# CodyRichter/MLMicroserviceTemplate

Hardware: AMD Instinct MI355X
Metric: requests/sec (whole node) + p50 latency, ResNet-50 bs=32 (higher is better)
Workload: dtype bf16; 1 GPU; model=resnet50-v1.5, global_batch=32, per_gpu_batch=32, image_size=224, parallelism=dp1, backend=fused, concurrent_slots=True, cu_partitions=2, hipgraph=True, inflight=4, numa_bound=True, partition_mode=intra, prestage=False, ranks_consistent=True, dist_backend=none, dist_world=1

## Files before the change

### mlmicroservicetemplate_amd/models/resnet.py

```python
from __future__ import annotations

import math
import os
from dataclasses import dataclass
from typing import Dict, List, Optional, Tuple

import torch
import torch.nn.functional as F

STAGES: Tuple[Tuple[int, int, int, int], ...] = (
    (3, 64, 256, 1),
    (4, 128, 512, 2),
    (6, 256, 1024, 2),
    (3, 512, 2048, 2),
)
IMAGENET_MEAN = (0.485 * 255, 0.456 * 255, 0.406 * 255)
IMAGENET_STD = (0.229 * 255, 0.224 * 255, 0.225 * 255)
NUM_CLASSES = 1000
CHAIN_CONV2_DEFAULT = ((64, 256, 64), (0, 256, 64))


@dataclass
class ConvSpec:
    name: str
    cin: int
    cout: int
    k: int
    stride: int
    pad: int


def conv_specs() -> List[ConvSpec]:
    specs = [ConvSpec("stem", 3, 64, 7, 2, 3)]
    cin = 64
    for si, (nblocks, mid, cout, stride) in enumerate(STAGES):
        for bi in range(nblocks):
            s = stride if bi == 0 else 1
            p = f"layer{si + 1}.{bi}"
            specs.append(ConvSpec(p + ".conv1", cin, mid, 1, 1, 0))
            specs.append(ConvSpec(p + ".conv2", mid, mid, 3, s, 1))
            specs.append(ConvSpec(p + ".conv3", mid, cout, 1, 1, 0))
            if bi == 0:
                specs.append(ConvSpec(p + ".down", cin, cout, 1, s, 0))
            cin = cout
    return specs


def init_resnet50(seed: int = 0, num_classes: int = NUM_CLASSES) -> Dict[str, torch.Tensor]:
    g = torch.Generator().manual_seed(seed)
    params: Dict[str, torch.Tensor] = {}
    for spec in conv_specs():
        fan_in = spec.cin * spec.k * spec.k
        w = torch.randn(spec.cout, spec.cin, spec.k, spec.k, generator=g) * math.sqrt(2.0 / fan_in)
        params[spec.name + ".w"] = w
        c = spec.cout
        params[spec.name + ".bn.gamma"] = 0.5 + 0.5 * torch.rand(c, generator=g)
        params[spec.name + ".bn.beta"] = 0.1 * torch.randn(c, generator=g)
        params[spec.name + ".bn.mean"] = 0.1 * torch.randn(c, generator=g)
        params[spec.name + ".bn.var"] = 0.5 + torch.rand(c, generator=g)
    params["fc.w"] = torch.randn(num_classes, 2048, generator=g) * math.sqrt(1.0 / 2048)
    params["fc.b"] = 0.01 * torch.randn(num_classes, generator=g)
    return params


_BN = {"weight": "gamma", "bias": "beta", "running_mean": "mean", "running_var": "var"}


def torchvision_name(k: str) -> Optional[str]:
    if k.endswith("num_batches_tracked"):
        return None
    p = k.split(".")
    if p[0] == "conv1":
        return "stem.w"
    if p[0] == "bn1":
        return f"stem.bn.{_BN[p[1]]}"
    if p[0] == "fc":
        return {"weight": "fc.w", "bias": "fc.b"}[p[1]]
    if p[0].startswith("layer") and len(p) >= 4:
        blk = f"{p[0]}.{p[1]}"
        if p[2].startswith("conv"):
            return f"{blk}.{p[2]}.w"
        if p[2].startswith("bn"):
            return f"{blk}.conv{p[2][2:]}.bn.{_BN[p[3]]}"
        if p[2] == "downsample":
            return f"{blk}.down.w" if p[3] == "0" else f"{blk}.down.bn.{_BN[p[4]]}"
    return k


def load_resnet50(path: str, num_classes: int = NUM_CLASSES) -> Dict[str, torch.Tensor]:
    from ..utils.checkpoint import load_validated

    spec = {k: (tuple(v.shape), torch.float32) for k, v in init_resnet50_spec(num_classes).items()}
    return load_validated(path, spec, rename=lambda k: k if k in spec else torchvision_name(k))


def init_resnet50_spec(num_classes: int = NUM_CLASSES) -> Dict[str, torch.Tensor]:
    out: Dict[str, torch.Tensor] = {}
    for spec in conv_specs():
        out[spec.name + ".w"] = torch.empty(spec.cout, spec.cin, spec.k, spec.k, device="meta")
        for n in ("gamma", "beta", "mean", "var"):
            out[f"{spec.name}.bn.{n}"] = torch.empty(spec.cout, device="meta")
    out["fc.w"] = torch.empty(num_classes, 2048, device="meta")
    out["fc.b"] = torch.empty(num_classes, device="meta")
    return out


BN_EPS = 1e-5


def fold_bn(params: Dict[str, torch.Tensor], name: str) -> Tuple[torch.Tensor, torch.Tensor]:
    gamma = params[name + ".bn.gamma"]
    beta = params[name + ".bn.beta"]
    mean = params[name + ".bn.mean"]
    var = params[name + ".bn.var"]
    scale = gamma / torch.sqrt(var + BN_EPS)
    bias = beta - mean * scale
    return scale, bias


def normalize_reference(images_u8_nhwc: torch.Tensor) -> torch.Tensor:
    x = images_u8_nhwc.float()
    mean = torch.tensor(IMAGENET_MEAN, device=x.device)
    std = torch.tensor(IMAGENET_STD, device=x.device)
    x = (x - mean) / std
    return x.permute(0, 3, 1, 2).contiguous()


def _ref_conv_bn(params, x, spec: ConvSpec, relu: bool, residual=None):
    y = F.conv2d(x, params[spec.name + ".w"], stride=spec.stride, padding=spec.pad)
    y = F.batch_norm(
        y,
        params[spec.name + ".bn.mean"],
        params[spec.name + ".bn.var"],
        params[spec.name + ".bn.gamma"],
        params[spec.name + ".bn.beta"],
        training=False,
        eps=BN_EPS,
    )
    if residual is not None:
        y = y + residual
    return F.relu(y) if relu else y


def resnet50_reference(params: Dict[str, torch.Tensor], images_u8_nhwc: torch.Tensor) -> torch.Tensor:
    specs = {s.name: s for s in conv_specs()}
    x = normalize_reference(images_u8_nhwc)
    x = _ref_conv_bn(params, x, specs["stem"], relu=True)
    x = F.max_pool2d(x, kernel_size=3, stride=2, padding=1)
    for si, (nblocks, _mid, _cout, _stride) in enumerate(STAGES):
        for bi in range(nblocks):
            p = f"layer{si + 1}.{bi}"
            identity = x
            if bi == 0:
                identity = _ref_conv_bn(params, x, specs[p + ".down"], relu=False)
            y = _ref_conv_bn(params, x, specs[p + ".conv1"], relu=True)
            y = _ref_conv_bn(params, y, specs[p + ".conv2"], relu=True)
            x = _ref_conv_bn(params, y, specs[p + ".conv3"], relu=True, residual=identity)
    x = x.mean(dim=(2, 3))
    return F.linear(x, params["fc.w"], params["fc.b"])


class ResNet50Eager(torch.nn.Module):

    def __init__(self, params: Dict[str, torch.Tensor], device, dtype=torch.bfloat16, fold: bool = True):
        super().__init__()
        self.specs = {s.name: s for s in conv_specs()}
        self.fold = fold
        self.dtype = dtype
        self.w: Dict[str, torch.Tensor] = {}
        self.sb: Dict[str, Tuple[torch.Tensor, torch.Tensor]] = {}
        for s in conv_specs():
            w = params[s.name + ".w"]
            scale, bias = fold_bn(params, s.name)
            if fold:
                w = w * scale.view(-1, 1, 1, 1)
            self.w[s.name] = w.to(device=device, dtype=dtype).contiguous(memory_format=torch.channels_last)
            self.sb[s.name] = (scale.to(device=device, dtype=dtype), bias.to(device=device, dtype=dtype))
        self.fc_w = params["fc.w"].to(device=device, dtype=dtype)
        self.fc_b = params["fc.b"].to(device=device, dtype=dtype)
        self.mean = torch.tensor(IMAGENET_MEAN, device=device, dtype=torch.float32)
        self.inv_std = 1.0 / torch.tensor(IMAGENET_STD, device=device, dtype=torch.float32)

    @torch.no_grad()
    def update_params(self, params: Dict[str, torch.Tensor]) -> None:
        for s in conv_specs():
            w = params[s.name + ".w"]
            scale, bias = fold_bn(params, s.name)
            if self.fold:
                w = w * scale.view(-1, 1, 1, 1)
            self.w[s.name].copy_(w)
            self.sb[s.name][0].copy_(scale)
            self.sb[s.name][1].copy_(bias)
        self.fc_w.copy_(params["fc.w"])
        self.fc_b.copy_(params["fc.b"])

    def _cbr(self, x, name, relu=True, residual=None):
        s = self.specs[name]
        y = F.conv2d(x, self.w[name], stride=s.stride, padding=s.pad)
        scale, bias = self.sb[name]
        if self.fold:
            y = y + bias.view(1, -1, 1, 1)
        else:
            y = y * scale.view(1, -1, 1, 1) + bias.view(1, -1, 1, 1)
        if residual is not None:
            y = y + residual
        return F.relu(y) if relu else y

    @torch.no_grad()
    def forward(self, images_u8_nhwc: torch.Tensor) -> torch.Tensor:
        x = ((images_u8_nhwc.float() - self.mean) * self.inv_std).to(self.dtype)
        x = x.permute(0, 3, 1, 2)
        x = self._cbr(x, "stem")
        x = F.max_pool2d(x, 3, 2, 1)
        for si, (nblocks, _m, _c, _s) in enumerate(STAGES):
            for bi in range(nblocks):
                p = f"layer{si + 1}.{bi}"
                identity = self._cbr(x, p + ".down", relu=False) if bi == 0 else x
                y = self._cbr(x, p + ".conv1")
                y = self._cbr(y, p + ".conv2")
                x = self._cbr(y, p + ".conv3", residual=identity)
        x = x.mean(dim=(2, 3))
        return F.linear(x, self.fc_w, self.fc_b)


def conv_shapes(image_size: int = 224) -> List[Tuple[ConvSpec, int, int]]:
    out: List[Tuple[ConvSpec, int, int]] = []
    block_in = cur = image_size
    for s in conv_specs():
        if s.name.endswith(".conv1"):
            block_in = cur
        hin = block_in if s.name.endswith(".down") else cur
        ho = (hin + 2 * s.pad - s.k) // s.stride + 1
        out.append((s, hin, ho))
        if s.name == "stem":
            cur = (ho + 2 - 3) // 2 + 1
        elif not s.name.endswith(".down"):
            cur = ho
    return out


def resnet50_flops_per_image(image_size: int = 224) -> float:
    total = 0.0
    for s, _hin, ho in conv_shapes(image_size):
        total += 2.0 * ho * ho * s.cout * s.cin * s.k * s.k
    return total + 2.0 * 2048 * NUM_CLASSES


class ResNet50Fused:

    def __init__(self, params: Dict[str, torch.Tensor], device, max_batch: int = 256,
                 tuning: Optional[Dict[str, Tuple[int, int]]] = None, image_size: int = 224):
        from .. import ops

        self.ops = ops
        self.device = torch.device(device)
        self.image_size = image_size
        self.tuning = dict(tuning or {})
        self.specs = {s.name: s for s in conv_specs()}
        self.w: Dict[str, torch.Tensor] = {}
        self.b: Dict[str, torch.Tensor] = {}
        for s in conv_specs():
            scale, bias = fold_bn(params, s.name)
            w = params[s.name + ".w"] * scale.view(-1, 1, 1, 1)
            self.w[s.name] = ops.pack_conv_weight(w).to(self.device)
            self.b[s.name] = bias.to(device=self.device, dtype=torch.float32).contiguous()
        self.dual_w: Dict[str, torch.Tensor] = {}
        self.dual_b: Dict[str, torch.Tensor] = {}
        for si, (_nb, _m, _c, _s) in enumerate(STAGES):
            p0 = f"layer{si + 1}.0"
            w3, wd = self.w[p0 + ".conv3"], self.w[p0 + ".down"]
            self.dual_w[p0] = torch.cat([w3.reshape(w3.shape[0], -1), wd.reshape(wd.shape[0], -1)], 1).contiguous()
            self.dual_b[p0] = (self.b[p0 + ".conv3"] + self.b[p0 + ".down"]).contiguous()
        self.fuse_down = True
        self.chain = os.environ.get("MLS_CHAIN", "1") != "0"
        self.chain_skip: set = {b for b in os.environ.get("MLS_CHAIN_SKIP", "").split(",") if b}
        mode = os.environ.get("MLS_CHAIN_CONV2", "1")
        self.chain_conv2 = mode != "0"
        self.chain_conv2_shapes = ops.CHAIN_CONV2_SHAPES if mode == "2" else CHAIN_CONV2_DEFAULT
        self.chain_conv2_skip: set = {b for b in os.environ.get("MLS_CHAIN_CONV2_SKIP", "").split(",") if b}
        self.chain_l3 = os.environ.get("MLS_CHAIN_L3", "0") == "1"
        if os.environ.get("MLS_CHAIN_L2_CW"):
            ops.set_chain_l2_cw(int(os.environ["MLS_CHAIN_L2_CW"]))
        if os.environ.get("MLS_CHAIN_L2_BM"):
            ops.lib().mls_chain_set_l2_bm(int(os.environ["MLS_CHAIN_L2_BM"]))
        if os.environ.get("MLS_CHAIN_VARIANT"):
            ops.lib().mls_chain_set_variant(int(os.environ["MLS_CHAIN_VARIANT"]))
        self.fuse_stem = image_size == 224 and os.environ.get("MLS_FUSED_STEM", "1") != "0"
        self.fuse_stem_conv1 = os.environ.get("MLS_STEM_CONV1", "0") == "1"
        self.fc_w = params["fc.w"].to(device=self.device, dtype=torch.bfloat16).contiguous()
        self.fc_b = params["fc.b"].to(device=self.device, dtype=torch.float32).contiguous()
        self.num_classes = self.fc_w.shape[0]
        self.mean = IMAGENET_MEAN
        self.std = IMAGENET_STD
        self.max_batch = max_batch
        self._ws = ops.StreamWorkspace(self._workspace_bytes(max_batch) // 4 + 1, self.device)
        self.fuse_head = os.environ.get("MLS_FUSED_HEAD", "1") != "0"
        self._pool = ops.StreamWorkspace(max_batch * self.fc_w.shape[1], self.device, zero=True)

    @property
    def workspace(self) -> torch.Tensor:
        return self._ws.get()

    @torch.no_grad()
    def update_params(self, params: Dict[str, torch.Tensor]) -> None:
        from .. import ops

        for s in conv_specs():
            scale, bias = fold_bn(params, s.name)
            w = ops.pack_conv_weight(params[s.name + ".w"] * scale.view(-1, 1, 1, 1))
            self.w[s.name].copy_(w)
            self.b[s.name].copy_(bias)
        for si in range(len(STAGES)):
            p0 = f"layer{si + 1}.0"
            w3, wd = self.w[p0 + ".conv3"], self.w[p0 + ".down"]
            self.dual_w[p0].copy_(torch.cat([w3.reshape(w3.shape[0], -1), wd.reshape(wd.shape[0], -1)], 1))
            self.dual_b[p0].copy_(self.b[p0 + ".conv3"] + self.b[p0 + ".down"])
        self.fc_w.copy_(params["fc.w"])
        self.fc_b.copy_(params["fc.b"])

    def layer_gemm_shapes(self, batch: int) -> List[Tuple[str, int, int, int]]:
        out = []
        for s, _hin, ho in conv_shapes(self.image_size):
            k = s.k * 32 if s.name == "stem" else s.k * s.k * s.cin
            out.append((s.name, batch * ho * ho, s.cout, k))
            if s.name.endswith(".0.down"):
                c3 = self.specs[s.name[: -len("down")] + "conv3"]
                out.append((s.name[: -len("down")] + "dual", batch * ho * ho, s.cout, c3.cin + s.cin))
        out.append(("fc", batch, self.num_classes, 2048))
        return out

    def _plan(self, name: str, M: int, N: int, K: int) -> Tuple[int, int]:
        if name in self.tuning:
            return self.tuning[name]
        return self.ops.gemm_heuristic(M, N, K)

    def _workspace_bytes(self, batch: int) -> int:
        need = 0
        for b in sorted({1, 2, 4, 8, 16, 32, 64, 128, 256, batch}):
            if b > batch:
                continue
            for name, M, N, K in self.layer_gemm_shapes(b):
                cfg, sk = self._plan(name, M, N, K)
                if cfg in self.ops.PIPE_CFGS:
                    sk = sk % 16 or 1
                if sk > 1:
                    need = max(need, sk * M * N * 4)
        return max(need, batch * NUM_CLASSES * 4, 1 << 20)

    def _conv(self, x, name, act, residual=None, pad=None):
        s = self.specs[name]
        cfg, sk = self.tuning.get(name, (0, 0))
        return self.ops.conv2d_nhwc(x, self.w[name], self.b[name], kernel=s.k, stride=s.stride,
                                    pad=s.pad if pad is None else pad,
                                    residual=residual, act=act, workspace=self.workspace, cfg=cfg, splitk=sk)


    def _chained(self, p: str, nxt: str, dual: bool) -> bool:
        if not self.chain or p in self.chain_skip:
            return False
        c3 = self.specs[p + ".conv3"]
        k = c3.cin + (self.specs[p + ".down"].cin if dual else 0)
        c1 = self.specs[nxt + ".conv1"]
        shape = (k, c3.cout, c1.cout)
        if shape == (256, 1024, 256) and not self.chain_l3:
            return False
        return c1.k == 1 and c1.stride == 1 and shape in self.ops.CHAIN_SHAPES

    def _conv2_fused(self, p: str, nxt: str, dual: bool, t1: torch.Tensor) -> bool:
        if not self.chain_conv2 or p in self.chain_conv2_skip:
            return False
        c2, c3 = self.specs[p + ".conv2"], self.specs[p + ".conv3"]
        kb = self.specs[p + ".down"].cin if dual else 0
        shape = (kb, c3.cout, self.specs[nxt + ".conv1"].cout)
        return (c2.k == 3 and c2.stride == 1 and c2.pad == 1 and c2.cin == 64 and c2.cout == 64
                and shape in self.chain_conv2_shapes and t1.shape[2] <= self.ops.CHAIN_CONV2_MAX_W)

    def forward(self, images_u8_nhwc: torch.Tensor) -> torch.Tensor:
        ops = self.ops
        B = images_u8_nhwc.shape[0]
        if self.fuse_head:
            pooled = self._trunk(images_u8_nhwc, pool=True)
            _v, _i, logits = ops.fc_head(pooled, self.fc_w, self.fc_b, 0, logits=self._logits_buf(B))
            return logits.to(torch.bfloat16)
        x = self._trunk(images_u8_nhwc, pool=False)
        pooled = ops.avgpool_global_nhwc(x)
        cfg, sk = self.tuning.get("fc", (0, 0))
        return ops.gemm(pooled, self.fc_w, self.fc_b, workspace=self.workspace, cfg=cfg, splitk=sk)

    __call__ = forward

    def _logits_buf(self, B: int) -> torch.Tensor:
        return self.workspace[: B * self.num_classes].view(B, self.num_classes)

    def classify(self, images_u8_nhwc: torch.Tensor, k: int = 5, err: Optional[torch.Tensor] = None):
        if self.fuse_head:
            pooled = self._trunk(images_u8_nhwc, pool=True)
            B = images_u8_nhwc.shape[0]
            vals, idx, _ = self.ops.fc_head(pooled, self.fc_w, self.fc_b, k, logits=self._logits_buf(B), err=err)
            return vals, idx
        vals, idx = self.ops.softmax_topk(self.forward(images_u8_nhwc), k)
        if err is not None:
            bad = (err[: idx.shape[0]] != 0).view(-1, 1)
            idx = torch.where(bad, torch.full_like(idx, -1), idx)
            vals = torch.where(bad, torch.full_like(vals, float("nan")), vals)
        return vals, idx

    def _trunk(self, images_u8_nhwc: torch.Tensor, pool: bool) -> torch.Tensor:
        ops = self.ops
        B = images_u8_nhwc.shape[0]
        if B > self.max_batch:
            raise ValueError(f"batch {B} > max_batch {self.max_batch}")
        if self.fuse_stem and self.fuse_stem_conv1:
            x, t1 = ops.stem_pool_u8(images_u8_nhwc, self.w["stem"], self.b["stem"], self.mean, self.std,
                                     conv1_w=self.w["layer1.0.conv1"], conv1_b=self.b["layer1.0.conv1"])
        else:
            if self.fuse_stem:
                x = ops.stem_pool_u8(images_u8_nhwc, self.w["stem"], self.b["stem"], self.mean, self.std)
            else:
                x = ops.normalize_u8(images_u8_nhwc, self.mean, self.std, pad=3)
                x = self._conv(x, "stem", ops.ACT_RELU, pad=0)
                x = ops.maxpool2d_nhwc(x, 3, 2, 1)
            t1 = self._conv(x, "layer1.0.conv1", ops.ACT_RELU)
        blocks = [(si, bi) for si, (nblocks, _m, _c, _s) in enumerate(STAGES) for bi in range(nblocks)]
        for idx, (si, bi) in enumerate(blocks):
            p = f"layer{si + 1}.{bi}"
            nxt = f"layer{blocks[idx + 1][0] + 1}.{blocks[idx + 1][1]}" if idx + 1 < len(blocks) else None
            dual = bi == 0 and self.fuse_down
            chained = nxt is not None and self._chained(p, nxt, dual)
            if chained and self._conv2_fused(p, nxt, dual, t1):
                w1n, b1n = self.w[nxt + ".conv1"], self.b[nxt + ".conv1"]
                w1n = w1n.reshape(w1n.shape[0], -1)
                w2, b2 = self.w[p + ".conv2"], self.b[p + ".conv2"]
                if dual:
                    x, t1 = ops.conv3x3_chain(t1, w2, b2, self.dual_w[p], self.dual_b[p], w1n, b1n, a2=x,
                                              stride2=self.specs[p + ".down"].stride)
                else:
                    w3 = self.w[p + ".conv3"]
                    x, t1 = ops.conv3x3_chain(t1, w2, b2, w3.reshape(w3.shape[0], -1), self.b[p + ".conv3"], w1n,
                                              b1n, residual=x)
                continue
            t2 = self._conv(t1, p + ".conv2", ops.ACT_RELU)
            if chained:
                w1n, b1n = self.w[nxt + ".conv1"], self.b[nxt + ".conv1"]
                w1n = w1n.reshape(w1n.shape[0], -1)
                if dual:
                    x, t1 = ops.conv1x1_chain(t2, self.dual_w[p], self.dual_b[p], w1n, b1n, a2=x,
                                              stride2=self.specs[p + ".down"].stride)
                else:
                    w3 = self.w[p + ".conv3"]
                    x, t1 = ops.conv1x1_chain(t2, w3.reshape(w3.shape[0], -1), self.b[p + ".conv3"], w1n, b1n,
                                              residual=x)
                continue
            if dual:
                cfg, sk = self.tuning.get(p + ".dual", (0, 0))
                x = ops.conv1x1_dual(t2, x, self.dual_w[p], self.dual_b[p], stride2=self.specs[p + ".down"].stride,
                                     act=ops.ACT_RELU, workspace=self.workspace, cfg=cfg, splitk=sk)
            else:
                identity = self._conv(x, p + ".down", ops.ACT_NONE) if bi == 0 else x
                if nxt is None and pool:
                    pooled = self._pool.get()[: B * self.fc_w.shape[1]].view(B, -1)
                    cfg, _sk = self.tuning.get(p + ".conv3", (0, 0))
                    s3 = self.specs[p + ".conv3"]
                    ops.conv2d_pool(t2, self.w[p + ".conv3"], self.b[p + ".conv3"], pooled, kernel=s3.k,
                                    stride=s3.stride, pad=s3.pad, residual=identity, act=ops.ACT_RELU, cfg=cfg)
                    return pooled
                x = self._conv(t2, p + ".conv3", ops.ACT_RELU, residual=identity)
            if nxt is not None:
                t1 = self._conv(x, nxt + ".conv1", ops.ACT_RELU)
        if pool:
            pooled = self._pool.get()[: B * self.fc_w.shape[1]].view(B, -1)
            pooled.copy_(ops.avgpool_global_nhwc(x).float())
            return pooled
        return x
```

### mlmicroservicetemplate_amd/ops/__init__.py

```python
from __future__ import annotations

from . import _lib
from ._lib import NativeError, available, check, lib, stream_ptr
from ._core import (
    ACT_GELU,
    ACT_NONE,
    ACT_RELU,
    ACT_SILU,
    ACT_SILU_MUL,
    ACT_TANH,
    StreamWorkspace,
    conv_out_hw,
)
from .tables import (
    gemm_plan,
    gemm_tile_plan,
    load_blas_tuning,
    small_m_plan_for,
    tile_cfg_for,
    tile_route_for,
)
from .gemm_ops import (
    FP8_MAX,
    GEMM_TILE_CFGS,
    SPLIT_COUNTER_ELEMS,
    fold_layernorm,
    fold_norm,
    fp8_reference,
    gemm,
    gemm_heuristic,
    gemm_rmsnorm,
    gemm_tile,
    gemm_tile_ln,
    layernorm_from_partials,
    ln_partials,
    interleave_gate_up,
    pack_skinny,
    pack_skinny_fp8,
    pack_skinny_reference,
    silu_mul_interleaved,
    skinny_fp8,
    mgemm,
    skinny_packed,
    skinny_packed_ar,
    split_counters,
)
from .dispatch import (
    BLAS_MIN_M,
    TILE_MIN_M,
    mgemm_route,
    linear_add_rmsnorm,
    linear,
    linear_ln,
    ln_foldable,
)
from .softmax import (
    softmax_rows,
    softmax_topk,
    topk_large,
)
from .vision import (
    CFG_HALO,
    CFG_HALO_N32,
    CFG_HALO_XL,
    CFG_PIPE,
    CHAIN_CONV2_MAX_W,
    CHAIN_CONV2_SHAPES,
    CHAIN_SHAPES,
    HALO_CFGS,
    PIPE_CFGS,
    PIPE_VARIANTS,
    avgpool_global_nhwc,
    bn_act,
    conv1x1_chain,
    conv1x1_dual,
    conv2d_nhwc,
    conv2d_pool,
    conv3x3_halo,
    conv3x3_halo_geometry,
    conv3x3_chain,
    conv3x3_pipe,
    conv3x3_pipe_geometry,
    fc_head,
    maxpool2d_nhwc,
    normalize_u8,
    pack_conv_weight,
    set_chain_l2_cw,
    stem_pool_u8,
)
from .transformer import (
    DecodePartials,
    decode_attention,
    decode_attention_fp8,
    decode_pick,
    embed_layernorm,
    embed_layernorm_packed,
    embedding,
    flash_attention,
    flash_attention_ctx,
    flash_attention_rows,
    kv_append,
    last_rows,
    layernorm,
    prefill_slots,
    rmsnorm,
    rope_,
    rope_kv_,
    rope_kv_fp8_,
    skinny_packed_combine,
    skinny_packed_combine_ar,
)
from .image import (
    IMAGE_CONTAINER_BYTES,
    IMAGE_SCRATCH_PER_IMAGE,
    d2h_push,
    gpu_sleep,
    h2d_pull,
    h2d_pull_cell,
    image_decode,
)
from .partition import (
    MASK_WORDS,
    census_cus,
    cu_census,
    cu_masked_stream,
    intra_partition_words,
    partition_masks,
    xcd_cu_masks,
)

__all__ = [
    "NativeError",
    "available",
    "lib",
    "conv2d_nhwc",
    "gemm",
    "normalize_u8",
    "maxpool2d_nhwc",
    "avgpool_global_nhwc",
    "bn_act",
    "softmax_topk",
    "softmax_rows",
    "pack_conv_weight",
    "conv_out_hw",
    "gemm_heuristic",
]
```

### mlmicroservicetemplate_amd/ops/_lib.py

```python
from __future__ import annotations

import ctypes
import os
import threading
from typing import Optional

import torch

from . import build as _build

_c = ctypes
_LOCK = threading.Lock()
_LIB: Optional[ctypes.CDLL] = None

P = _c.c_void_p
I = _c.c_int
L = _c.c_long
F = _c.c_float
SZ = _c.c_size_t
FP = _c.POINTER(_c.c_float)

_SIGS = {
    "mls_conv2d": [P, P, P, P, P, P, P, SZ, I, I, I, I, I, I, I, I, I, I, I, I, P],
    "mls_conv2d_dual": [P, P, P, P, P, P, SZ, I, I, I, I, I, I, I, I, I, I, I, I, P],
    "mls_conv_chain": [P, P, P, P, P, P, P, P, P, I, I, I, I, I, I, I, I, I, I, P],
    "mls_conv_chain_conv2": [P, P, P, P, P, P, P, P, P, P, P, I, I, I, I, I, I, I, I, I, I, P],
    "mls_gemm": [P, P, P, P, P, P, P, SZ, I, I, I, I, I, I, P],
    "mls_gemm_heuristic": [I, I, I, _c.POINTER(I), _c.POINTER(I)],
    "mls_gemm_tile": [P, P, P, P, P, I, I, I, I, I, I, I, I, I, P, _c.c_longlong, P, I, P],
    "mls_gemm_tile_pick": [I, I],
    "mls_gemm_tile_ln": [P, P, P, P, P, I, I, I, I, I, P, P, P, P, _c.c_longlong, F, P],
    "mls_gemm_num_cfgs": [],
    "mls_normalize_u8": [P, P, I, I, I, I, FP, FP, P],
    "mls_maxpool2d": [P, P, I, I, I, I, I, I, I, P],
    "mls_stem_pool": [P, P, P, P, I, I, I, FP, FP, P],
    "mls_stem_pool_conv1": [P, P, P, P, I, I, I, FP, FP, P, P, P, P],
    "mls_conv3x3_halo": [P, P, P, P, P, P, SZ, I, I, I, I, I, I, I, I, P],
    "mls_conv3x3_halo_geometry": [I, I, I, _c.POINTER(I), _c.POINTER(I)],
    "mls_conv3x3_halo_geometry_v": [I, I, I, I, _c.POINTER(I), _c.POINTER(I)],
    "mls_conv2d_pool": [P, P, P, P, P, P, P, I, I, I, I, I, I, I, I, I, I, I, I, P],
    "mls_fc_head": [P, P, P, P, P, P, P, I, I, I, I, I, P, _c.c_longlong, P],
    "mls_conv3x3_pipe": [P, P, P, P, P, SZ, I, I, I, I, I, I, I, I, I, P],
    "mls_conv3x3_pipe_geometry": [I, I, I, I, _c.POINTER(I), _c.POINTER(I)],
    "mls_conv3x3_pipe_num_variants": [],
    "mls_avgpool_global": [P, P, I, I, I, P],
    "mls_bn_act": [P, P, P, P, L, I, I, P],
    "mls_silu_mul_interleaved": [P, P, L, I, P],
    "mls_softmax_topk": [P, I, P, P, I, I, I, I, F, P],
    "mls_softmax_rows": [P, P, P, I, I, I, F, P],
    "mls_topk_merge": [P, P, P, P, I, I, I, I, I, I, P],
    "mls_topk_chunks": [P, P, P, I, I, I, I, I, P],
    "mls_layernorm": [P, P, P, P, P, P, L, I, F, I, P],
    "mls_embed_ln": [P, P, P, P, P, P, P, P, L, I, I, I, F, P],
    "mls_embed_ln2": [P, P, I, P, P, P, P, P, P, P, P, L, I, I, I, F, P],
    "mls_embedding": [P, P, P, L, I, I, I, P],
    "mls_prefill_slots": [P, P, P, P, I, I, I, I, I, P, P],
    "mls_last_rows": [P, P, P, I, I, I, P, P, P],
    "mls_rope": [P, P, P, P, L, I, I, I, P],
    "mls_ar_create": [I, I, L, P],
    "mls_ar_create2": [I, I, L, L, P],
    "mls_ar_allreduce2": [P, P, P, L, _c.c_longlong, P],
    "mls_ar_handle": [P, P],
    "mls_ar_handle_size": [],
    "mls_ar_open": [P, P],
    "mls_ar_allreduce": [P, P, P, L, _c.c_longlong, P],
    "mls_ar_error": [P, P],
    "mls_ar_error_peek": [P, P, P],
    "mls_ar_set_timeout": [P, _c.c_longlong],
    "mls_ar_allgather": [P, P, P, L, _c.c_longlong, P],
    "mls_ar_reset": [P],
    "mls_gpu_sleep": [L, P],
    "mls_h2d_pull": [P, P, _c.c_longlong, I, P],
    "mls_h2d_pull_cell": [P, P, _c.c_longlong, I, P],
    "mls_d2h_push": [P, P, _c.c_longlong, I, P],
    "mls_stem_set_stamps": [P],
    "mls_stem_set_version": [I],
    "mls_flash_set_version": [I],
    "mls_image_decode": [P, P, P, L, I, P, P],
    "mls_decode_pick": [P, P, I, I, I, P, P, P, P, P, P, P, I, P, P, P, P, P],
    "mls_ar_destroy": [P],
    "mls_rope_kv": [P, P, P, P, L, I, I, I, I, P, P, P, P, I, I, L, I, I, P],
    "mls_kv_append": [P, I, I, I, P, P, P, L, I, I, I, P],
    "mls_rope_kv_fp8": [P, P, P, P, L, I, I, I, I, P, P, P, P, P, P, I, I, L, I, I, P],
    "mls_decode_attention_fp8": [P, P, P, P, P, P, P, P, P, I, I, I, P, P, P, P, I, I, I, I, I, I, I, F, P, I, I, I,
                                 P],
    "mls_flash_attention": [P, P, P, P, I, I, I, I, I, I, I, I, I, P, I, F, P],
    "mls_flash_attention_rows": [P, P, P, P, I, I, I, I, I, I, I, I, I, I, P, I, F, P],
    "mls_flash_attention_ctx": [P, P, P, P, I, I, P, P, P, P, I, I, I, I, I, I, I, L, I, F, P],
    "mls_skinny_gemm": [P, P, P, P, P, P, SZ, I, I, I, I, I, P],
    "mls_mgemm": [P, P, P, P, P, P, SZ, I, I, I, I, I, I, P], "mls_mgemm_auto_split": [I, I, I],
    "mls_gemm_slabs": [P, P, P, SZ, I, I, I, I, I, P, P], "mls_splitk_add_rmsnorm": [P, SZ, I, I, I, P, P, P, F, P],
    "mls_skinny_gemm_norm": [P, P, P, P, P, P, P, P, SZ, I, I, I, I, I, I, F, P],
    "mls_skinny_pack": [P, P, I, I, P],
    "mls_skinny_packed": [P, P, P, P, P, P, P, I, I, I, I, I, F, I, P],
    "mls_decode_attention": [P, P, P, P, P, P, P, I, I, L, P, P, P, P, I, I, I, I, I, I, I, F, P, I, I, I, I, P],
    "mls_skinny_packed_combine": [P, P, P, P, I, I, I, I, P, P, P, P, I, I, I, I, I, P],
    "mls_skinny_packed_ar": [P, P, P, P, P, I, I, I, I, F, I, P, P],
    "mls_skinny_packed_combine_ar": [P, P, P, P, I, I, I, I, P, P, I, I, I, I, P, P],
    "mls_skinny_fp8": [P, P, P, P, P, P, P, P, I, I, I, I, I, F, I, P],
    "mls_stream_create_cumask": [P, I, _c.POINTER(P)],
    "mls_stream_get_cumask": [P, P, I],
    "mls_stream_destroy": [P],
    "mls_cu_census": [P, I, I, P],
}
_OPTIONAL_SIGS: dict = {"mls_set_debug_flags": [I], "mls_chain_set_l2_cw": [I],
    "mls_chain_set_l2_bm": [I], "mls_chain_set_variant": [I], "mls_chain_set_grid": [I],
    "mls_engine_launch": [P, P, P, _c.c_longlong, P, I, P, P, P, P, P], "mls_engine_launch_after": [P, P, P, P, _c.c_longlong, P, I, P, P, P, P, P], "mls_skinny_set_variant": [I], "mls_skinny_set_max_split": [I]}


class NativeError(RuntimeError):
    pass


def register_signatures(sigs: dict, optional: bool = False) -> None:
    (_OPTIONAL_SIGS if optional else _SIGS).update(sigs)
    if _LIB is not None:
        _bind(_LIB)


def _bind(lib: ctypes.CDLL) -> None:
    for name, argtypes in list(_SIGS.items()) + list(_OPTIONAL_SIGS.items()):
        fn = getattr(lib, name, None)
        if fn is None:
            if name in _SIGS:
                raise NativeError(f"{name} missing from {lib._name}; rebuild the kernels")
            continue
        fn.argtypes = argtypes
        fn.restype = _c.c_int


DEBUG = os.environ.get("MLS_DEBUG", "0") == "1"
DEBUG_TUS = ("attention", "norm_ops", "stem_pool", "conv3x3_halo", "kv_fp8", "flash_ctx")
DEBUG_CODES = {
    101: "rope/KV append: cache slot beyond the cache",
    102: "rope/KV append: position beyond the RoPE table",
    201: "decode attention: lens[b] exceeds the split grid (host context bound max_len too small)",
    202: "decode attention (rope mode): position outside the RoPE table or != lens - 1",
    203: "decode attention (fp8 cache): page id outside the pool",
    301: "flash attention: kv_lens[b] > S",
    311: "flash attention (ctx): not 0 <= past[b] <= lens[b] <= the rows of a slot",
    312: "flash attention (ctx): slot outside the cache",
    313: "flash attention (ctx): page id outside the pool",
}


def lib(build_if_missing: bool = True) -> ctypes.CDLL:
    global _LIB
    if _LIB is not None:
        return _LIB
    with _LOCK:
        if _LIB is not None:
            return _LIB
        path = _build.lib_path(DEBUG)
        override = os.environ.get("MLS_LIB_OVERRIDE")
        if override:
            build_if_missing = False
            path = override
        if build_if_missing:
            try:
                path = _build.build(debug=DEBUG)
            except Exception as e:
                if not os.path.exists(path):
                    raise NativeError(f"native kernels unavailable and build failed: {e}") from e
        if not os.path.exists(path):
            raise NativeError(f"native kernel library not built: {path}")
        handle = ctypes.CDLL(path, mode=ctypes.RTLD_GLOBAL)
        _bind(handle)
        _LIB = handle
        return _LIB


def available() -> bool:
    try:
        lib()
        return True
    except Exception:
        return False


def check(rc: int, what: str) -> None:
    if rc != 0:
        raise NativeError(f"{what} failed with status {rc}")
    if DEBUG and not torch.cuda.is_current_stream_capturing():
        debug_check(what)


def debug_check(what: str = "kernel") -> None:
    if not DEBUG:
        return
    torch.cuda.synchronize()
    buf = (_c.c_int * 4)()
    for tu in DEBUG_TUS:
        fn = getattr(lib(), f"mls_debug_read_{tu}", None)
        if fn is None:
            raise NativeError(f"{lib()._name} is not a debug build")
        fn.argtypes = [_c.c_void_p]
        fn.restype = _c.c_int
        if fn(_c.cast(buf, _c.c_void_p)) != 0:
            raise NativeError("mls_debug_read failed")
        if buf[0]:
            raise NativeError(f"{what}: bound violated [{buf[0]}] {DEBUG_CODES.get(buf[0], '?')} "
                              f"(block {buf[1]},{buf[2]} thread {buf[3]})")


def stream_ptr(device: Optional[torch.device] = None) -> int:
    return torch.cuda.current_stream(device).cuda_stream
```

### mlmicroservicetemplate_amd/ops/csrc/conv_chain.hip

```cpp
#include "common.h"
#include "fastdiv.h"

namespace {

#define LDS3 __attribute__((address_space(3)))

MLS_DEV void glds16(rsrc_t r, char* lds, int voff, int soff) {
  __builtin_amdgcn_raw_ptr_buffer_load_lds(r, (LDS3 void*)lds, 16, voff, soff, 0, 0);
}

typedef unsigned int u32x4v __attribute__((__vector_size__(16)));

MLS_DEV uint32_t lds_off(const void* p);
MLS_DEV u32x4v lds_ld16_issue(uint32_t off);
template <typename T>
MLS_DEV void lds_landed(T& v);

#define CONST4 __attribute__((address_space(4)))

MLS_DEV f32x4 bias4(const float* b, int nt0, int fq) {
  if (!b) return f32x4{0.f, 0.f, 0.f, 0.f};
  const CONST4 f32x4* bp = (const CONST4 f32x4*)(b + nt0);
  const f32x4 b0 = bp[0], b1 = bp[1], b2 = bp[2], b3 = bp[3];
  return fq == 0 ? b0 : fq == 1 ? b1 : fq == 2 ? b2 : b3;
}

struct ChainArgs {
  const bf16* a1;
  const bf16* a2;
  const bf16* w3;
  const float* b3;
  const bf16* res;
  bf16* y;
  const bf16* w1;
  const float* b1;
  bf16* t1;
  int M, Ka, Kb, N1, N2;
  int Ho, Wo, H2, W2, stride2;
  FastDiv fd_howo, fd_wo;
  uint32_t a1_bytes, a2_bytes, w3_bytes, res_bytes, y_bytes, w1_bytes, t1_bytes;
  const bf16* t1in;
  const bf16* w2;
  const float* b2;
  uint32_t t1in_bytes, w2_bytes;
};

template <int CPR>
MLS_DEV int row_swz(int r) {
  if constexpr (CPR == 8) return r & 7;
  else return (r & 1) | ((r >> 1) & 2);
}

template <int BM, int KS, int N1, int N2, int CW, int OCC, bool SW, bool C2 = false>
__global__ __launch_bounds__(512, OCC) void conv_chain_kernel(const ChainArgs a) {
  constexpr int NW = 8, NT = 512, WM = 4, WN = 2;
  constexpr int WTM = BM / WM, TM = WTM / 16;
  constexpr int TN = CW / WN / 16;
  constexpr int TN2 = N2 / WN / 16;
  constexpr int CPR = CW / 8;
  constexpr int RPP = 64 / CPR;
  constexpr int A1_BYTES = BM * KS * 128;
  constexpr int W3_BYTES = CW * KS * 128;
  constexpr int W1_BYTES = N2 * CW * 2;
  constexpr int R_BYTES = BM * CW * 2;
  constexpr int STAGE = W3_BYTES + W1_BYTES + R_BYTES;
  constexpr int EPI_BYTES = BM * N2 * 2;
  constexpr int RING = A1_BYTES + 2 * STAGE;
  constexpr int LDS_BYTES = RING > EPI_BYTES ? RING : EPI_BYTES;
  constexpr int A1_PW = BM / 8 * KS / NW;
  constexpr int A1_S0 = C2 ? 1 : 0;
  constexpr int A1_PWL = BM / 8 * (KS - A1_S0) / NW;
  constexpr int W3_PW = CW / 8 * KS / NW;
  constexpr int W1_PW = N2 / RPP / NW;
  constexpr int R_PW = BM / RPP / NW;
  constexpr int Y_ST = BM * CPR / NT;
  constexpr int T_ST = BM * N2 / 8 / NT;
  constexpr int NJ = N1 / CW;
  static_assert(TM >= 1 && TN >= 1 && TN2 >= 1 && (CW == 64 || CW == 32), "tile");
  static_assert(A1_PW * NW * 8 == BM * KS && W3_PW * NW * 8 == CW * KS, "A1 / W3 DMA split");
  static_assert(W1_PW * NW * RPP == N2 && R_PW * NW * RPP == BM, "W1 / residual DMA split");
  static_assert(Y_ST * NT == BM * CPR && T_ST * NT == BM * N2 / 8, "epilogue split");
  static_assert(LDS_BYTES <= 160 * 1024, "LDS");
  __shared__ __attribute__((aligned(16))) char smem[LDS_BYTES];

  const int tid = threadIdx.x, lane = tid & 63;
  const int wid = __builtin_amdgcn_readfirstlane(tid >> 6);
  const int wm = wid / WN, wn = wid % WN;
  const int fr = lane & 15, fq = lane >> 4;
  const int m0 = xcd_remap(blockIdx.x, gridDim.x) * BM;
  const int K1 = a.Ka + a.Kb, KSA = a.Ka / 64;
  const bool has_res = a.res != nullptr;

  float b3v[SW ? 1 : NJ][TN], b1v[TN2];
  if constexpr (!SW) {
#pragma unroll
    for (int j = 0; j < NJ; ++j)
#pragma unroll
      for (int jn = 0; jn < TN; ++jn) b3v[j][jn] = a.b3 ? a.b3[j * CW + wn * (CW / 2) + jn * 16 + fr] : 0.f;
#pragma unroll
    for (int jn = 0; jn < TN2; ++jn) b1v[jn] = a.b1 ? a.b1[wn * (N2 / 2) + jn * 16 + fr] : 0.f;
  }

  const int r8 = lane >> 3, lc = (lane & 7) ^ r8;
  const int rq = lane / CPR, lq = (lane % CPR) ^ row_swz<CPR>(rq);

  const rsrc_t a1r = make_rsrc(a.a1, a.a1_bytes);
  const rsrc_t a2r = make_rsrc(a.a2, a.a2_bytes);
  const rsrc_t w3r = make_rsrc(a.w3, a.w3_bytes);
  const rsrc_t w1r = make_rsrc(a.w1, a.w1_bytes);
  const rsrc_t rr = make_rsrc(a.res, a.res_bytes);
  const rsrc_t yr = make_rsrc(a.y, a.y_bytes);
  const rsrc_t tr = make_rsrc(a.t1, a.t1_bytes);

  char* const sA1 = smem;
  auto stage_base = [&](int buf) { return smem + A1_BYTES + buf * STAGE; };

#pragma unroll
  for (int i = 0; i < A1_PWL; ++i) {
    const int q = A1_S0 * (BM / 8) + wid * A1_PWL + i;
    const int s = q / (BM / 8), rb = q - s * (BM / 8);
    const int m = m0 + rb * 8 + r8;
    char* dst = sA1 + q * 1024;
    if (s < KSA) {
      glds16(a1r, dst, m < a.M ? (m * a.Ka + s * 64 + lc * 8) * 2 : OOB, 0);
    } else {
      int off = OOB;
      if (m < a.M) {
        const int b = fastdiv(m, a.fd_howo), rem = m - b * (a.Ho * a.Wo);
        const int oh = fastdiv(rem, a.fd_wo), ow = rem - oh * a.Wo;
        off = (((b * a.H2 + oh * a.stride2) * a.W2 + ow * a.stride2) * a.Kb + (s - KSA) * 64 + lc * 8) * 2;
      }
      glds16(a2r, dst, off, 0);
    }
  }

  auto issue = [&](int j, int buf) {
    char* sW3 = stage_base(buf);
    char* sW1 = sW3 + W3_BYTES;
    char* sR = sW1 + W1_BYTES;
#pragma unroll
    for (int i = 0; i < W3_PW; ++i) {
      const int q = wid * W3_PW + i;
      const int s = q / (CW / 8), rb = q - s * (CW / 8);
      glds16(w3r, sW3 + q * 1024, ((j * CW + rb * 8 + r8) * K1 + s * 64 + lc * 8) * 2, 0);
    }
#pragma unroll
    for (int i = 0; i < W1_PW; ++i) {
      const int q = wid * W1_PW + i;
      glds16(w1r, sW1 + q * 1024, ((q * RPP + rq) * N1 + j * CW + lq * 8) * 2, 0);
    }
    if (has_res) {
#pragma unroll
      for (int i = 0; i < R_PW; ++i) {
        const int q = wid * R_PW + i;
        const int m = m0 + q * RPP + rq;
        glds16(rr, sR + q * 1024, m < a.M ? (m * N1 + j * CW + lq * 8) * 2 : OOB, 0);
      }
    }
  };

  if constexpr (C2) {
    constexpr int TAPS = 9, TSLOTS = 4, TAHEAD = 3, SROWS = 256, TNP = 64 / WN / 16;
    static_assert(BM == 128 && STAGE >= SROWS * 128 && STAGE >= TSLOTS * 8192, "strip / tap ring alias one stage each");
    char* const sS = stage_base(0);
    char* const sT = stage_base(1);
    const rsrc_t t1r = make_rsrc(a.t1in, a.t1in_bytes);
    const rsrc_t w2r = make_rsrc(a.w2, a.w2_bytes);
    const int halo = a.Wo + 1;
#pragma unroll
    for (int i = 0; i < SROWS / 8 / NW; ++i) {
      const int q = wid * (SROWS / 8 / NW) + i;
      const int sr = q * 8 + r8, p = m0 - halo + sr;
      glds16(t1r, sS + q * 1024, (p >= 0 && p < a.M && sr < BM + 2 * halo) ? (p * 64 + lc * 8) * 2 : OOB, 0);
    }
    auto issue_tap = [&](int t) {
      glds16(w2r, sT + (t % TSLOTS) * 8192 + wid * 1024, (((wid * 8 + r8) * TAPS + t) * 64 + lc * 8) * 2, 0);
    };
#pragma unroll
    for (int t = 0; t < TAHEAD; ++t) issue_tap(t);

    int okm[TM];
#pragma unroll
    for (int i = 0; i < TM; ++i) {
      const int m = m0 + wm * WTM + i * 16 + fr;
      okm[i] = 0;
      if (m < a.M) {
        const int b = fastdiv(m, a.fd_howo), rem = m - b * (a.Ho * a.Wo);
        const int oh = fastdiv(rem, a.fd_wo), ow = rem - oh * a.Wo;
#pragma unroll
        for (int t = 0; t < TAPS; ++t)
          if ((unsigned)(oh + t / 3 - 1) < (unsigned)a.Ho && (unsigned)(ow + t % 3 - 1) < (unsigned)a.Wo)
            okm[i] |= 1 << t;
      }
    }

    f32x4 accp[TM][TNP];
#pragma unroll
    for (int i = 0; i < TM; ++i)
#pragma unroll
      for (int jn = 0; jn < TNP; ++jn) accp[i][jn] = f32x4{0.f, 0.f, 0.f, 0.f};
#pragma unroll
    for (int t = 0; t < TAPS; ++t) {
      if (t + 2 < TAPS) asm volatile("s_waitcnt vmcnt(2)" ::: "memory");
      else if (t + 1 < TAPS) asm volatile("s_waitcnt vmcnt(1)" ::: "memory");
      else asm volatile("s_waitcnt vmcnt(0)" ::: "memory");
      asm volatile("s_waitcnt lgkmcnt(0)" ::: "memory");
      __builtin_amdgcn_s_barrier();
      if (t + TAHEAD < TAPS) issue_tap(t + TAHEAD);
      const int shift = halo + (t / 3 - 1) * a.Wo + (t % 3 - 1);
      const uint32_t oS = lds_off(sS), oT = lds_off(sT + (t % TSLOTS) * 8192);
      u32x4v av[2][TM], bv[2][TNP];
#pragma unroll
      for (int kk = 0; kk < 2; ++kk) {
        const int ch = fq + 4 * kk;
#pragma unroll
        for (int i = 0; i < TM; ++i) {
          const int r = wm * WTM + i * 16 + fr + shift;
          av[kk][i] = lds_ld16_issue(oS + (r * 8 + (ch ^ (r & 7))) * 16);
        }
#pragma unroll
        for (int jn = 0; jn < TNP; ++jn) {
          const int n = wn * 32 + jn * 16 + fr;
          bv[kk][jn] = lds_ld16_issue(oT + (n * 8 + (ch ^ (n & 7))) * 16);
        }
      }
#pragma unroll
      for (int kk = 0; kk < 2; ++kk) {
#pragma unroll
        for (int i = 0; i < TM; ++i) lds_landed(av[kk][i]);
#pragma unroll
        for (int jn = 0; jn < TNP; ++jn) lds_landed(bv[kk][jn]);
      }
#pragma unroll
      for (int kk = 0; kk < 2; ++kk) {
        bf16x8 af[TM], bfv[TNP];
#pragma unroll
        for (int i = 0; i < TM; ++i) {
          u32x4v v = av[kk][i];
          if (!((okm[i] >> t) & 1)) v = u32x4v{0u, 0u, 0u, 0u};
          af[i] = __builtin_bit_cast(bf16x8, v);
        }
#pragma unroll
        for (int jn = 0; jn < TNP; ++jn) bfv[jn] = __builtin_bit_cast(bf16x8, bv[kk][jn]);
#pragma unroll
        for (int i = 0; i < TM; ++i)
#pragma unroll
          for (int jn = 0; jn < TNP; ++jn)
            accp[i][jn] = __builtin_amdgcn_mfma_f32_16x16x32_bf16(bfv[jn], af[i], accp[i][jn], 0, 0, 0);
      }
    }
#pragma unroll
    for (int jn = 0; jn < TNP; ++jn) {
      const int nt0 = wn * 32 + jn * 16, col = nt0 + fq * 4;
      const f32x4 bb = bias4(a.b2, nt0, fq);
#pragma unroll
      for (int i = 0; i < TM; ++i) {
        const int row = wm * WTM + i * 16 + fr;
        bf16x4 q;
#pragma unroll
        for (int r = 0; r < 4; ++r) {
          const float e = accp[i][jn][r];
          q[r] = (bf16)fmaxf(e + bb[r], 0.f);
        }
        *reinterpret_cast<uint2*>(sA1 + row * 128 + (((col >> 3) ^ (row & 7)) << 4) + (col & 7) * 2) =
            __builtin_bit_cast(uint2, q);
      }
    }
    asm volatile("s_waitcnt lgkmcnt(0)" ::: "memory");
    __builtin_amdgcn_s_barrier();
  }
  issue(0, 0);

  f32x4 acc2[TM][TN2];
#pragma unroll
  for (int i = 0; i < TM; ++i)
#pragma unroll
    for (int jn = 0; jn < TN2; ++jn) acc2[i][jn] = f32x4{0.f, 0.f, 0.f, 0.f};

#pragma unroll
  for (int j = 0; j < NJ; ++j) {
    if (j == 0) {
      asm volatile("s_waitcnt vmcnt(0)" ::: "memory");
      if constexpr (!SW) {
#pragma unroll
        for (int jj = 0; jj < NJ; ++jj)
#pragma unroll
          for (int jn = 0; jn < TN; ++jn) asm volatile("" ::"v"(b3v[jj][jn]));
#pragma unroll
        for (int jn = 0; jn < TN2; ++jn) asm volatile("" ::"v"(b1v[jn]));
      }
    } else {
      asm volatile("s_waitcnt vmcnt(%0)" ::"n"(Y_ST) : "memory");
    }
    asm volatile("s_waitcnt lgkmcnt(0)" ::: "memory");
    __builtin_amdgcn_s_barrier();
    if (j + 1 < NJ) issue(j + 1, (j + 1) & 1);
    char* sW3 = stage_base(j & 1);
    char* sW1 = sW3 + W3_BYTES;
    char* sR = sW1 + W1_BYTES;

    f32x4 acc1[TM][TN];
#pragma unroll
    for (int i = 0; i < TM; ++i)
#pragma unroll
      for (int jn = 0; jn < TN; ++jn) acc1[i][jn] = f32x4{0.f, 0.f, 0.f, 0.f};
    const uint4* A1s = reinterpret_cast<const uint4*>(sA1);
    const uint4* W3s = reinterpret_cast<const uint4*>(sW3);
#pragma unroll
    for (int kk = 0; kk < 2 * KS; ++kk) {
      const int s = kk >> 1, ch = fq + 4 * (kk & 1);
      bf16x8 af[TM], bfv[TN];
#pragma unroll
      for (int i = 0; i < TM; ++i) {
        const int r = wm * WTM + i * 16 + fr;
        af[i] = __builtin_bit_cast(bf16x8, A1s[s * BM * 8 + r * 8 + (ch ^ (r & 7))]);
      }
#pragma unroll
      for (int jn = 0; jn < TN; ++jn) {
        const int n = wn * (CW / 2) + jn * 16 + fr;
        bfv[jn] = __builtin_bit_cast(bf16x8, W3s[s * CW * 8 + n * 8 + (ch ^ (n & 7))]);
      }
#pragma unroll
      for (int i = 0; i < TM; ++i)
#pragma unroll
        for (int jn = 0; jn < TN; ++jn)
          acc1[i][jn] = SW ? __builtin_amdgcn_mfma_f32_16x16x32_bf16(bfv[jn], af[i], acc1[i][jn], 0, 0, 0)
                                       : __builtin_amdgcn_mfma_f32_16x16x32_bf16(af[i], bfv[jn], acc1[i][jn], 0, 0, 0);
    }

    if constexpr (SW) {
#pragma unroll
      for (int jn = 0; jn < TN; ++jn) {
        const int nt0 = wn * (CW / 2) + jn * 16, col = nt0 + fq * 4;
        const f32x4 bb = bias4(a.b3, j * CW + nt0, fq);
#pragma unroll
        for (int i = 0; i < TM; ++i) {
          const int row = wm * WTM + i * 16 + fr;
          uint2* p = reinterpret_cast<uint2*>(sR + row * (CW * 2) + (((col >> 3) ^ row_swz<CPR>(row)) << 4) +
                                              (col & 7) * 2);
          float rs[4] = {0.f, 0.f, 0.f, 0.f};
          if (has_res) {
            const bf16x4 rv = __builtin_bit_cast(bf16x4, *p);
#pragma unroll
            for (int r = 0; r < 4; ++r) rs[r] = (float)rv[r];
          }
          bf16x4 q;
#pragma unroll
          for (int r = 0; r < 4; ++r) {
            const float e = acc1[i][jn][r];
            q[r] = (bf16)fmaxf(e + bb[r] + rs[r], 0.f);
          }
          *p = __builtin_bit_cast(uint2, q);
        }
      }
    } else
#pragma unroll
    for (int jn = 0; jn < TN; ++jn) {
      const int col = wn * (CW / 2) + jn * 16 + fr;
      const float bb = b3v[j][jn];
#pragma unroll
      for (int i = 0; i < TM; ++i)
#pragma unroll
        for (int r = 0; r < 4; ++r) {
          const int row = wm * WTM + i * 16 + fq * 4 + r;
          bf16* p = reinterpret_cast<bf16*>(sR + row * (CW * 2) + (((col >> 3) ^ row_swz<CPR>(row)) << 4) +
                                            (col & 7) * 2);
          const float e = acc1[i][jn][r];
          float v = e + bb;
          if (has_res) v += (float)*p;
          *p = (bf16)fmaxf(v, 0.f);
        }
    }
    asm volatile("s_waitcnt lgkmcnt(0)" ::: "memory");
    __builtin_amdgcn_s_barrier();

#pragma unroll
    for (int it = 0; it < Y_ST; ++it) {
      const int q = tid + it * NT;
      const int row = q / CPR, c = q % CPR;
      const uint4 v = *reinterpret_cast<const uint4*>(sR + row * (CW * 2) + ((c ^ row_swz<CPR>(row)) << 4));
      const int m = m0 + row;
      __builtin_amdgcn_raw_buffer_store_b128(__builtin_bit_cast(u32x4v, v), yr,
                                             m < a.M ? (m * N1 + j * CW + c * 8) * 2 : OOB, 0, 0);
    }

    const uint4* Ys = reinterpret_cast<const uint4*>(sR);
    const uint4* W1s = reinterpret_cast<const uint4*>(sW1);
#pragma unroll
    for (int kk = 0; kk < CW / 32; ++kk) {
      const int ch = fq + 4 * kk;
      bf16x8 af[TM], bfv[TN2];
#pragma unroll
      for (int i = 0; i < TM; ++i) {
        const int r = wm * WTM + i * 16 + fr;
        af[i] = __builtin_bit_cast(bf16x8, Ys[r * CPR + (ch ^ row_swz<CPR>(r))]);
      }
#pragma unroll
      for (int jn = 0; jn < TN2; ++jn) {
        const int n = wn * (N2 / 2) + jn * 16 + fr;
        bfv[jn] = __builtin_bit_cast(bf16x8, W1s[n * CPR + (ch ^ row_swz<CPR>(n))]);
      }
#pragma unroll
      for (int i = 0; i < TM; ++i)
#pragma unroll
        for (int jn = 0; jn < TN2; ++jn)
          acc2[i][jn] = SW ? __builtin_amdgcn_mfma_f32_16x16x32_bf16(bfv[jn], af[i], acc2[i][jn], 0, 0, 0)
                                       : __builtin_amdgcn_mfma_f32_16x16x32_bf16(af[i], bfv[jn], acc2[i][jn], 0, 0, 0);
    }
  }

  asm volatile("s_waitcnt lgkmcnt(0)" ::: "memory");
  __builtin_amdgcn_s_barrier();
  constexpr int TPR = N2 / 8;
  bf16* to = reinterpret_cast<bf16*>(smem);
  if constexpr (SW) {
#pragma unroll
    for (int jn = 0; jn < TN2; ++jn) {
      const int nt0 = wn * (N2 / 2) + jn * 16, col = nt0 + fq * 4;
      const f32x4 bb = bias4(a.b1, nt0, fq);
#pragma unroll
      for (int i = 0; i < TM; ++i) {
        const int row = wm * WTM + i * 16 + fr;
        bf16x4 q;
#pragma unroll
        for (int r = 0; r < 4; ++r) {
          const float e = acc2[i][jn][r];
          q[r] = (bf16)fmaxf(e + bb[r], 0.f);
        }
        *reinterpret_cast<uint2*>(to + row * N2 + ((((col >> 3) ^ (row & 7))) << 3) + (col & 7)) =
            __builtin_bit_cast(uint2, q);
      }
    }
  } else
#pragma unroll
  for (int jn = 0; jn < TN2; ++jn) {
    const int col = wn * (N2 / 2) + jn * 16 + fr;
    const float bb = b1v[jn];
#pragma unroll
    for (int i = 0; i < TM; ++i)
#pragma unroll
      for (int r = 0; r < 4; ++r) {
        const int row = wm * WTM + i * 16 + fq * 4 + r;
        const float e = acc2[i][jn][r];
        to[row * N2 + ((((col >> 3) ^ (row & 7))) << 3) + (col & 7)] = (bf16)fmaxf(e + bb, 0.f);
      }
  }
  asm volatile("s_waitcnt lgkmcnt(0)" ::: "memory");
  __builtin_amdgcn_s_barrier();
#pragma unroll
  for (int it = 0; it < T_ST; ++it) {
    const int q = tid + it * NT;
    const int row = q / TPR, c = q - (q / TPR) * TPR;
    const uint4 v = *reinterpret_cast<const uint4*>(to + row * N2 + ((c ^ (row & 7)) << 3));
    const int m = m0 + row;
    __builtin_amdgcn_raw_buffer_store_b128(__builtin_bit_cast(u32x4v, v), tr, m < a.M ? (m * a.N2 + c * 8) * 2 : OOB,
                                           0, 0);
  }
}

MLS_DEV void vm_wait(int n) {
#define MLS_VMW(k) \
  case k: asm volatile("s_waitcnt vmcnt(" #k ")" ::: "memory"); break;
  switch (n) {
    MLS_VMW(1) MLS_VMW(2) MLS_VMW(3) MLS_VMW(4) MLS_VMW(5) MLS_VMW(6) MLS_VMW(7) MLS_VMW(8) MLS_VMW(9) MLS_VMW(10)
    MLS_VMW(11) MLS_VMW(12) MLS_VMW(13) MLS_VMW(14) MLS_VMW(15) MLS_VMW(16) MLS_VMW(17) MLS_VMW(18) MLS_VMW(19)
    MLS_VMW(20)
    default: asm volatile("s_waitcnt vmcnt(0)" ::: "memory");
  }
#undef MLS_VMW
}

MLS_DEV uint32_t lds_off(const void* p) { return (uint32_t)(uintptr_t)(LDS3 const char*)p; }
MLS_DEV uint2 lds_ld8_issue(uint32_t off) {
  uint2 v;
  asm volatile("ds_read_b64 %0, %1" : "=v"(v) : "v"(off) : "memory");
  return v;
}
MLS_DEV uint32_t lds_ld2_issue(uint32_t off) {
  uint32_t v;
  asm volatile("ds_read_u16 %0, %1" : "=v"(v) : "v"(off) : "memory");
  return v;
}
template <typename T>
MLS_DEV void lds_landed(T& v) { asm volatile("s_waitcnt lgkmcnt(0)" : "+v"(v)::"memory"); }
MLS_DEV u32x4v lds_ld16_issue(uint32_t off) {
  u32x4v v;
  asm volatile("ds_read_b128 %0, %1" : "=v"(v) : "v"(off) : "memory");
  return v;
}
MLS_DEV uint4 lds_ld16(uint32_t off) {
  uint4 v;
  asm volatile("ds_read_b128 %0, %1\n\ts_waitcnt lgkmcnt(0)" : "=v"(v) : "v"(off) : "memory");
  return v;
}
MLS_DEV void lds_st8(uint32_t off, uint2 v) { asm volatile("ds_write_b64 %0, %1" ::"v"(off), "v"(v) : "memory"); }
MLS_DEV void lds_st2(uint32_t off, bf16 h) {
  const uint32_t v = __builtin_bit_cast(unsigned short, h);
  asm volatile("ds_write_b16 %0, %1" ::"v"(off), "v"(v) : "memory");
}

template <int BM, int KS, int N1, int N2, int CW, int S, int OCC, bool SW, bool PERS>
__global__ __launch_bounds__(512, OCC) void conv_chain_ring_kernel(const ChainArgs a, const int ntiles) {
  constexpr int NW = 8, NT = 512, WM = 4, WN = 2;
  constexpr int WTM = BM / WM, TM = WTM / 16;
  constexpr int TN = CW / WN / 16;
  constexpr int TN2 = N2 / WN / 16;
  constexpr int CPR = CW / 8;
  constexpr int RPP = 64 / CPR;
  constexpr int NJ = N1 / CW;
  constexpr int A1_BYTES = BM * KS * 128;
  constexpr int W3_BYTES = CW * KS * 128;
  constexpr int W1_BYTES = N2 * CW * 2;
  constexpr int R_BYTES = BM * CW * 2;
  constexpr int EPI_BYTES = BM * N2 * 2;
  constexpr int STAGE = PERS ? R_BYTES : W3_BYTES + W1_BYTES + R_BYTES;
  constexpr int OFF_W3 = (PERS ? 2 : 1) * A1_BYTES;
  constexpr int OFF_W1 = OFF_W3 + (PERS ? NJ * W3_BYTES : 0);
  constexpr int OFF_EPI = OFF_W1 + (PERS ? NJ * W1_BYTES : 0);
  constexpr int OFF_RING = OFF_EPI + (PERS ? EPI_BYTES : 0);
  constexpr int RING_END = OFF_RING + S * STAGE;
  constexpr int LDS_BYTES = RING_END > EPI_BYTES ? RING_END : EPI_BYTES;
  constexpr int A1_P = BM / 8 * KS, W3_P = CW / 8 * KS, W1_P = N2 / RPP, R_P = BM / RPP;
  constexpr int Y_ST = BM * CPR / NT;
  constexpr int T_ST = BM * N2 / 8 / NT;
  static_assert(TM >= 1 && TN >= 1 && TN2 >= 1 && (CW == 64 || CW == 32), "tile");
  static_assert(S >= 2 && S - 1 <= NJ && (!PERS || NJ % S == 0), "ring depth");
  static_assert(Y_ST * NT == BM * CPR && T_ST * NT == BM * N2 / 8, "epilogue split");
  static_assert(LDS_BYTES <= 160 * 1024, "LDS");
  __shared__ __attribute__((aligned(16))) char smem[LDS_BYTES];

  const int tid = threadIdx.x, lane = tid & 63;
  const int wid = __builtin_amdgcn_readfirstlane(tid >> 6);
  const int wm = wid / WN, wn = wid % WN;
  const int fr = lane & 15, fq = lane >> 4;
  const int G = gridDim.x;
  int tile = chain_first_tile(blockIdx.x, G);
  if (tile >= ntiles) return;
  int m0 = tile * BM;
  const int K1 = a.Ka + a.Kb, KSA = a.Ka / 64;
  const bool has_res = a.res != nullptr;

  float b3v[SW ? 1 : NJ][TN], b1v[TN2];
  if constexpr (!SW) {
#pragma unroll
    for (int j = 0; j < NJ; ++j)
#pragma unroll
      for (int jn = 0; jn < TN; ++jn) b3v[j][jn] = a.b3 ? a.b3[j * CW + wn * (CW / 2) + jn * 16 + fr] : 0.f;
#pragma unroll
    for (int jn = 0; jn < TN2; ++jn) b1v[jn] = a.b1 ? a.b1[wn * (N2 / 2) + jn * 16 + fr] : 0.f;
  }

  const int r8 = lane >> 3, lc = (lane & 7) ^ r8;
  const int rq = lane / CPR, lq = (lane % CPR) ^ row_swz<CPR>(rq);

  const rsrc_t a1r = make_rsrc(a.a1, a.a1_bytes);
  const rsrc_t a2r = make_rsrc(a.a2, a.a2_bytes);
  const rsrc_t w3r = make_rsrc(a.w3, a.w3_bytes);
  const rsrc_t w1r = make_rsrc(a.w1, a.w1_bytes);
  const rsrc_t rr = make_rsrc(a.res, a.res_bytes);
  const rsrc_t yr = make_rsrc(a.y, a.y_bytes);
  const rsrc_t tr = make_rsrc(a.t1, a.t1_bytes);

  auto pieces = [&](int P) { return P / NW + (wid < P % NW ? 1 : 0); };
  const int n_a1 = pieces(A1_P);
  const int n_st = (PERS ? 0 : pieces(W3_P) + pieces(W1_P)) + (has_res ? pieces(R_P) : 0);

  auto issue_a1 = [&](int mt, char* dstA) {
#pragma unroll
    for (int i = 0; i < (A1_P + NW - 1) / NW; ++i) {
      const int q = i * NW + wid;
      if (A1_P % NW != 0 && q >= A1_P) break;
      const int s = q / (BM / 8), rb = q - s * (BM / 8);
      const int m = mt + rb * 8 + r8;
      char* dst = dstA + q * 1024;
      if (s < KSA) {
        glds16(a1r, dst, m < a.M ? (m * a.Ka + s * 64 + lc * 8) * 2 : OOB, 0);
      } else {
        int off = OOB;
        if (m < a.M) {
          const int b = fastdiv(m, a.fd_howo), rem = m - b * (a.Ho * a.Wo);
          const int oh = fastdiv(rem, a.fd_wo), ow = rem - oh * a.Wo;
          off = (((b * a.H2 + oh * a.stride2) * a.W2 + ow * a.stride2) * a.Kb + (s - KSA) * 64 + lc * 8) * 2;
        }
        glds16(a2r, dst, off, 0);
      }
    }
  };
  auto issue_w = [&](int j, char* sW3, char* sW1) {
#pragma unroll
    for (int i = 0; i < (W3_P + NW - 1) / NW; ++i) {
      const int q = i * NW + wid;
      if (W3_P % NW != 0 && q >= W3_P) break;
      const int s = q / (CW / 8), rb = q - s * (CW / 8);
      glds16(w3r, sW3 + q * 1024, ((j * CW + rb * 8 + r8) * K1 + s * 64 + lc * 8) * 2, 0);
    }
#pragma unroll
    for (int i = 0; i < (W1_P + NW - 1) / NW; ++i) {
      const int q = i * NW + wid;
      if (W1_P % NW != 0 && q >= W1_P) break;
      glds16(w1r, sW1 + q * 1024, ((q * RPP + rq) * N1 + j * CW + lq * 8) * 2, 0);
    }
  };
  auto issue_r = [&](int j, int mt, char* sR) {
    if (!has_res) return;
#pragma unroll
    for (int i = 0; i < (R_P + NW - 1) / NW; ++i) {
      const int q = i * NW + wid;
      if (R_P % NW != 0 && q >= R_P) break;
      const int m = mt + q * RPP + rq;
      glds16(rr, sR + q * 1024, m < a.M ? (m * N1 + j * CW + lq * 8) * 2 : OOB, 0);
    }
  };
  auto w3_at = [&](int j, int slot) { return smem + (PERS ? OFF_W3 + j * W3_BYTES : OFF_RING + slot * STAGE); };
  auto w1_at = [&](int j, int slot) {
    return smem + (PERS ? OFF_W1 + j * W1_BYTES : OFF_RING + slot * STAGE + W3_BYTES);
  };
  auto r_at = [&](int slot) { return smem + OFF_RING + slot * STAGE + (PERS ? 0 : W3_BYTES + W1_BYTES); };
  auto issue_stage = [&](int j, int slot, int mt) {
    if constexpr (!PERS) issue_w(j, w3_at(j, slot), w1_at(j, slot));
    issue_r(j, mt, r_at(slot));
  };

  if constexpr (PERS) {
#pragma unroll
    for (int j = 0; j < NJ; ++j) issue_w(j, w3_at(j, 0), w1_at(j, 0));
  }
  issue_a1(m0, smem);
#pragma unroll
  for (int s = 0; s < S - 1; ++s) issue_stage(s, s, m0);
  if constexpr (PERS) {
    asm volatile("s_waitcnt vmcnt(0)" ::: "memory");
    if constexpr (!SW) {
#pragma unroll
      for (int jj = 0; jj < NJ; ++jj)
#pragma unroll
        for (int jn = 0; jn < TN; ++jn) asm volatile("" ::"v"(b3v[jj][jn]));
#pragma unroll
      for (int jn = 0; jn < TN2; ++jn) asm volatile("" ::"v"(b1v[jn]));
    }
  }

  f32x4 acc2[TM][TN2];
#pragma unroll
  for (int i = 0; i < TM; ++i)
#pragma unroll
    for (int jn = 0; jn < TN2; ++jn) acc2[i][jn] = f32x4{0.f, 0.f, 0.f, 0.f};

  int abuf = 0;
  bool first = true;
  for (;;) {
    int m0n = a.M;
    if constexpr (PERS) {
      const int next = chain_next_tile(tile, G);
      if (next < ntiles) m0n = next * BM;
    }
    char* const sA1 = smem + abuf * A1_BYTES;

#pragma unroll
    for (int j = 0; j < NJ; ++j) {
      if constexpr (PERS) {
        const int jm = j < S - 1 ? j : S - 1;
        const int ahead = (S - 2) * n_st + (j >= NJ - S + 2 ? n_a1 : 0);
        vm_wait(ahead + (first ? jm * Y_ST : (S - 1) * Y_ST + (j <= S - 2 ? T_ST : 0)));
      } else {
        const int left = NJ - 1 - j < S - 2 ? NJ - 1 - j : S - 2;
        const int jm = j < S - 1 ? j : S - 1;
        vm_wait(left * n_st + jm * Y_ST);
        if (!SW && j == 0) {
#pragma unroll
          for (int jj = 0; jj < NJ; ++jj)
#pragma unroll
            for (int jn = 0; jn < TN; ++jn) asm volatile("" ::"v"(b3v[jj][jn]));
#pragma unroll
          for (int jn = 0; jn < TN2; ++jn) asm volatile("" ::"v"(b1v[jn]));
        }
      }
      asm volatile("s_waitcnt lgkmcnt(0)" ::: "memory");
      __builtin_amdgcn_s_barrier();
      {
        const int jn = j + S - 1;
        if (jn < NJ) {
          issue_stage(jn, jn % S, m0);
        } else if (PERS) {
          if (jn == NJ) issue_a1(m0n, smem + (abuf ^ 1) * A1_BYTES);
          issue_stage(jn - NJ, jn % S, m0n);
        }
      }
      char* const sW3 = w3_at(j, j % S);
      char* const sW1 = w1_at(j, j % S);
      char* const sR = r_at(j % S);

      f32x4 acc1[TM][TN];
#pragma unroll
      for (int i = 0; i < TM; ++i)
#pragma unroll
        for (int jn = 0; jn < TN; ++jn) acc1[i][jn] = f32x4{0.f, 0.f, 0.f, 0.f};
      const uint4* A1s = reinterpret_cast<const uint4*>(sA1);
      const uint4* W3s = reinterpret_cast<const uint4*>(sW3);
#pragma unroll
      for (int kk = 0; kk < 2 * KS; ++kk) {
        const int s = kk >> 1, ch = fq + 4 * (kk & 1);
        bf16x8 af[TM], bfv[TN];
#pragma unroll
        for (int i = 0; i < TM; ++i) {
          const int r = wm * WTM + i * 16 + fr;
          af[i] = __builtin_bit_cast(bf16x8, A1s[s * BM * 8 + r * 8 + (ch ^ (r & 7))]);
        }
#pragma unroll
        for (int jn = 0; jn < TN; ++jn) {
          const int n = wn * (CW / 2) + jn * 16 + fr;
          bfv[jn] = __builtin_bit_cast(bf16x8, W3s[s * CW * 8 + n * 8 + (ch ^ (n & 7))]);
        }
#pragma unroll
        for (int i = 0; i < TM; ++i)
#pragma unroll
          for (int jn = 0; jn < TN; ++jn)
            acc1[i][jn] = SW ? __builtin_amdgcn_mfma_f32_16x16x32_bf16(bfv[jn], af[i], acc1[i][jn], 0, 0, 0)
                             : __builtin_amdgcn_mfma_f32_16x16x32_bf16(af[i], bfv[jn], acc1[i][jn], 0, 0, 0);
      }

      auto y_at = [&](int row, int col) {
        return lds_off(sR + row * (CW * 2) + (((col >> 3) ^ row_swz<CPR>(row)) << 4) + (col & 7) * 2);
      };
      if constexpr (SW) {
        uint2 rv[TN][TM];
        if (has_res) {
#pragma unroll
          for (int jn = 0; jn < TN; ++jn)
#pragma unroll
            for (int i = 0; i < TM; ++i)
              rv[jn][i] = lds_ld8_issue(y_at(wm * WTM + i * 16 + fr, wn * (CW / 2) + jn * 16 + fq * 4));
#pragma unroll
          for (int jn = 0; jn < TN; ++jn)
#pragma unroll
            for (int i = 0; i < TM; ++i) lds_landed(rv[jn][i]);
        }
#pragma unroll
        for (int jn = 0; jn < TN; ++jn) {
          const int nt0 = wn * (CW / 2) + jn * 16, col = nt0 + fq * 4;
          const f32x4 bb = bias4(a.b3, j * CW + nt0, fq);
#pragma unroll
          for (int i = 0; i < TM; ++i) {
            const int row = wm * WTM + i * 16 + fr;
            float rs[4] = {0.f, 0.f, 0.f, 0.f};
            if (has_res) {
              const bf16x4 r4 = __builtin_bit_cast(bf16x4, rv[jn][i]);
#pragma unroll
              for (int r = 0; r < 4; ++r) rs[r] = (float)r4[r];
            }
            bf16x4 q;
#pragma unroll
            for (int r = 0; r < 4; ++r) {
              const float e = acc1[i][jn][r];
              q[r] = (bf16)fmaxf(e + bb[r] + rs[r], 0.f);
            }
            lds_st8(y_at(row, col), __builtin_bit_cast(uint2, q));
          }
        }
      } else {
        uint32_t rv[TN][TM][4];
        if (has_res) {
#pragma unroll
          for (int jn = 0; jn < TN; ++jn)
#pragma unroll
            for (int i = 0; i < TM; ++i)
#pragma unroll
              for (int r = 0; r < 4; ++r)
                rv[jn][i][r] = lds_ld2_issue(y_at(wm * WTM + i * 16 + fq * 4 + r, wn * (CW / 2) + jn * 16 + fr));
#pragma unroll
          for (int jn = 0; jn < TN; ++jn)
#pragma unroll
            for (int i = 0; i < TM; ++i)
#pragma unroll
              for (int r = 0; r < 4; ++r) lds_landed(rv[jn][i][r]);
        }
#pragma unroll
        for (int jn = 0; jn < TN; ++jn) {
          const int col = wn * (CW / 2) + jn * 16 + fr;
          const float bb = b3v[j][jn];
#pragma unroll
          for (int i = 0; i < TM; ++i)
#pragma unroll
            for (int r = 0; r < 4; ++r) {
              const int row = wm * WTM + i * 16 + fq * 4 + r;
              const float e = acc1[i][jn][r];
              float v = e + bb;
              if (has_res) v += (float)__builtin_bit_cast(bf16, (unsigned short)rv[jn][i][r]);
              lds_st2(y_at(row, col), (bf16)fmaxf(v, 0.f));
            }
        }
      }
      asm volatile("s_waitcnt lgkmcnt(0)" ::: "memory");
      __builtin_amdgcn_s_barrier();

#pragma unroll
      for (int it = 0; it < Y_ST; ++it) {
        const int q = tid + it * NT;
        const int row = q / CPR, c = q % CPR;
        const uint4 v = lds_ld16(lds_off(sR + row * (CW * 2) + ((c ^ row_swz<CPR>(row)) << 4)));
        const int m = m0 + row;
        __builtin_amdgcn_raw_buffer_store_b128(__builtin_bit_cast(u32x4v, v), yr,
                                               m < a.M ? (m * N1 + j * CW + c * 8) * 2 : OOB, 0, 0);
      }

      const uint4* Ys = reinterpret_cast<const uint4*>(sR);
      const uint4* W1s = reinterpret_cast<const uint4*>(sW1);
#pragma unroll
      for (int kk = 0; kk < CW / 32; ++kk) {
        const int ch = fq + 4 * kk;
        bf16x8 af[TM], bfv[TN2];
#pragma unroll
        for (int i = 0; i < TM; ++i) {
          const int r = wm * WTM + i * 16 + fr;
          af[i] = __builtin_bit_cast(bf16x8, Ys[r * CPR + (ch ^ row_swz<CPR>(r))]);
        }
#pragma unroll
        for (int jn = 0; jn < TN2; ++jn) {
          const int n = wn * (N2 / 2) + jn * 16 + fr;
          bfv[jn] = __builtin_bit_cast(bf16x8, W1s[n * CPR + (ch ^ row_swz<CPR>(n))]);
        }
#pragma unroll
        for (int i = 0; i < TM; ++i)
#pragma unroll
          for (int jn = 0; jn < TN2; ++jn)
            acc2[i][jn] = SW ? __builtin_amdgcn_mfma_f32_16x16x32_bf16(bfv[jn], af[i], acc2[i][jn], 0, 0, 0)
                             : __builtin_amdgcn_mfma_f32_16x16x32_bf16(af[i], bfv[jn], acc2[i][jn], 0, 0, 0);
      }
    }

    constexpr int TPR = N2 / 8;
    bf16* to = reinterpret_cast<bf16*>(smem + (PERS ? OFF_EPI : 0));
    if constexpr (!PERS) {
      asm volatile("s_waitcnt lgkmcnt(0)" ::: "memory");
      __builtin_amdgcn_s_barrier();
    }
    if constexpr (SW) {
#pragma unroll
      for (int jn = 0; jn < TN2; ++jn) {
        const int nt0 = wn * (N2 / 2) + jn * 16, col = nt0 + fq * 4;
        const f32x4 bb = bias4(a.b1, nt0, fq);
#pragma unroll
        for (int i = 0; i < TM; ++i) {
          const int row = wm * WTM + i * 16 + fr;
          bf16x4 q;
#pragma unroll
          for (int r = 0; r < 4; ++r) {
            const float e = acc2[i][jn][r];
            q[r] = (bf16)fmaxf(e + bb[r], 0.f);
          }
          lds_st8(lds_off(to + row * N2 + ((((col >> 3) ^ (row & 7))) << 3) + (col & 7)), __builtin_bit_cast(uint2, q));
        }
      }
    } else {
#pragma unroll
      for (int jn = 0; jn < TN2; ++jn) {
        const int col = wn * (N2 / 2) + jn * 16 + fr;
        const float bb = b1v[jn];
#pragma unroll
        for (int i = 0; i < TM; ++i)
#pragma unroll
          for (int r = 0; r < 4; ++r) {
            const int row = wm * WTM + i * 16 + fq * 4 + r;
            const float e = acc2[i][jn][r];
            lds_st2(lds_off(to + row * N2 + ((((col >> 3) ^ (row & 7))) << 3) + (col & 7)), (bf16)fmaxf(e + bb, 0.f));
          }
      }
    }
    asm volatile("s_waitcnt lgkmcnt(0)" ::: "memory");
    __builtin_amdgcn_s_barrier();
#pragma unroll
    for (int it = 0; it < T_ST; ++it) {
      const int q = tid + it * NT;
      const int row = q / TPR, c = q - (q / TPR) * TPR;
      const uint4 v = lds_ld16(lds_off(to + row * N2 + ((c ^ (row & 7)) << 3)));
      const int m = m0 + row;
      __builtin_amdgcn_raw_buffer_store_b128(__builtin_bit_cast(u32x4v, v), tr,
                                             m < a.M ? (m * a.N2 + c * 8) * 2 : OOB, 0, 0);
    }
    if constexpr (!PERS) break;
    tile = chain_next_tile(tile, G);
    if (tile >= ntiles) break;
    m0 = m0n;
    abuf ^= 1;
    first = false;
#pragma unroll
    for (int i = 0; i < TM; ++i)
#pragma unroll
      for (int jn = 0; jn < TN2; ++jn) acc2[i][jn] = f32x4{0.f, 0.f, 0.f, 0.f};
  }
  if constexpr (PERS) asm volatile("s_waitcnt vmcnt(0)" ::: "memory");
}

template <int KS, int N1, int N2, int CW, int BM = 128, bool C2 = false>
int launch_chain(const ChainArgs& a, hipStream_t st) {
  constexpr int LDS = BM * KS * 128 + 2 * (CW * KS * 128 + N2 * CW * 2 + BM * CW * 2);
  constexpr int OCC = LDS <= 80 * 1024 ? 4 : 2;
#ifdef MLS_CHAIN_SWAP
  constexpr bool SW = MLS_CHAIN_SWAP;
#else
  constexpr bool SW = KS == 1;
#endif
  hipLaunchKernelGGL((conv_chain_kernel<BM, KS, N1, N2, CW, OCC, SW, C2>), dim3((unsigned)((a.M + BM - 1) / BM)),
                     dim3(512), 0, st, a);
  return (int)hipGetLastError();
}

int g_chain_grid = 0;

template <int BM, int KS, int N1, int N2, int CW, int S, bool PERS>
int launch_ring(const ChainArgs& a, hipStream_t st) {
#ifdef MLS_CHAIN_SWAP
  constexpr bool SW = MLS_CHAIN_SWAP;
#else
  constexpr bool SW = KS == 1;
#endif
  constexpr int LDS = PERS ? 2 * BM * KS * 128 + N1 * KS * 128 + N2 * N1 * 2 + BM * N2 * 2 + S * BM * CW * 2
                            : BM * KS * 128 + S * (CW * KS * 128 + N2 * CW * 2 + BM * CW * 2);
  constexpr int OCC = LDS <= 80 * 1024 ? 4 : 2;
  const int ntiles = (a.M + BM - 1) / BM;
  int grid = ntiles;
  if (PERS) {
    const int cus = mls_num_cus();
    grid = g_chain_grid > 0 ? g_chain_grid : (ntiles < cus ? ntiles : cus);
  }
  hipLaunchKernelGGL((conv_chain_ring_kernel<BM, KS, N1, N2, CW, S, OCC, SW, PERS>), dim3((unsigned)grid), dim3(512), 0,
                     st, a, ntiles);
  return (int)hipGetLastError();
}

int g_chain_cw_l2 = 0;
int g_chain_bm_l2 = 128;
int g_chain_variant = 0;

constexpr bool RING_L1_DUAL = false, RING_L2 = true, RING_L2_OUT = false;

bool use_ring(bool shape_default) { return g_chain_variant == 2 || (g_chain_variant == 0 && shape_default); }

}

extern "C" {

int mls_conv_chain(const void* a1, const void* a2, const void* w3, const float* b3, const void* res, void* y,
                   const void* w1, const float* b1, void* t1, int B, int Ho, int Wo, int Ka, int H2, int W2, int Kb,
                   int stride2, int N1, int N2, void* stream) {
  if (B <= 0 || Ho <= 0 || Wo <= 0 || Ka <= 0 || Ka % 64 || Kb < 0 || Kb % 64 || N1 <= 0 || N1 % 64 || N2 <= 0)
    return MLS_BAD_ARG;
  if (Kb > 0 && (stride2 < 1 || (Ho - 1) * stride2 >= H2 || (Wo - 1) * stride2 >= W2 || res)) return MLS_BAD_ARG;
  ChainArgs a{};
  a.a1 = (const bf16*)a1;
  a.a2 = (const bf16*)a2;
  a.w3 = (const bf16*)w3;
  a.b3 = b3;
  a.res = (const bf16*)res;
  a.y = (bf16*)y;
  a.w1 = (const bf16*)w1;
  a.b1 = b1;
  a.t1 = (bf16*)t1;
  a.M = B * Ho * Wo;
  a.Ka = Ka;
  a.Kb = Kb;
  a.N1 = N1;
  a.N2 = N2;
  a.Ho = Ho, a.Wo = Wo, a.H2 = H2, a.W2 = W2, a.stride2 = stride2;
  a.fd_howo = fastdiv_make((uint32_t)(Ho * Wo));
  a.fd_wo = fastdiv_make((uint32_t)Wo);
  const long M = a.M;
  const long sizes[7] = {M * Ka * 2, (long)B * H2 * W2 * Kb * 2, (long)N1 * (Ka + Kb) * 2, res ? M * N1 * 2 : 0,
                         M * N1 * 2, (long)N2 * N1 * 2, M * N2 * 2};
  for (long s : sizes)
    if (s >= 0x7fffffffL) return MLS_UNSUPPORTED;
  a.a1_bytes = (uint32_t)sizes[0];
  a.a2_bytes = (uint32_t)sizes[1];
  a.w3_bytes = (uint32_t)sizes[2];
  a.res_bytes = (uint32_t)sizes[3];
  a.y_bytes = (uint32_t)sizes[4];
  a.w1_bytes = (uint32_t)sizes[5];
  a.t1_bytes = (uint32_t)sizes[6];
  const hipStream_t st = (hipStream_t)stream;
  const int ks = (Ka + Kb) / 64;
  if (ks == 1 && N1 == 256 && N2 == 64) return launch_chain<1, 256, 64, 64>(a, st);
  if (ks == 2 && N1 == 256 && N2 == 64)
    return use_ring(RING_L1_DUAL) ? launch_ring<64, 2, 256, 64, 64, 2, true>(a, st)
                                  : launch_chain<2, 256, 64, 64>(a, st);
  if (ks == 1 && N1 == 256 && N2 == 128) return launch_chain<1, 256, 128, 64>(a, st);
  const bool l2_override = g_chain_variant == 0 && (g_chain_bm_l2 == 64 || g_chain_cw_l2 != 0);
  if (ks == 2 && N1 == 512 && N2 == 128) {
    if (!l2_override && use_ring(RING_L2)) return launch_ring<128, 2, 512, 128, 64, 2, false>(a, st);
    if (g_chain_bm_l2 == 64) return launch_chain<2, 512, 128, 64, 64>(a, st);
    return g_chain_cw_l2 == 32 ? launch_chain<2, 512, 128, 32>(a, st) : launch_chain<2, 512, 128, 64>(a, st);
  }
  if (ks == 2 && N1 == 512 && N2 == 256) {
    if (!l2_override && use_ring(RING_L2_OUT)) return launch_ring<128, 2, 512, 256, 32, 3, false>(a, st);
    return g_chain_bm_l2 == 64 ? launch_chain<2, 512, 256, 64, 64>(a, st) : launch_chain<2, 512, 256, 32>(a, st);
  }
  if (ks == 4 && N1 == 1024 && N2 == 256) return launch_chain<4, 1024, 256, 32>(a, st);
  return MLS_UNSUPPORTED;
}

int mls_conv_chain_conv2(const void* t1_in, const void* w2, const float* b2, const void* a2, const void* w3,
                         const float* b3, const void* res, void* y, const void* w1, const float* b1, void* t1, int B,
                         int H, int W, int Ka, int H2, int W2, int Kb, int stride2, int N1, int N2, void* stream) {
  if (B <= 0 || H <= 0 || W <= 0 || Ka <= 0 || Kb < 0 || Kb % 64 || N1 <= 0 || N1 % 64 || N2 <= 0) return MLS_BAD_ARG;
  if (Kb > 0 && (stride2 < 1 || (H - 1) * stride2 >= H2 || (W - 1) * stride2 >= W2 || res)) return MLS_BAD_ARG;
  if (Ka != 64 || 2 * (W + 1) + 128 > 256) return MLS_UNSUPPORTED;
  ChainArgs a{};
  a.t1in = (const bf16*)t1_in;
  a.w2 = (const bf16*)w2;
  a.b2 = b2;
  a.a2 = (const bf16*)a2;
  a.w3 = (const bf16*)w3;
  a.b3 = b3;
  a.res = (const bf16*)res;
  a.y = (bf16*)y;
  a.w1 = (const bf16*)w1;
  a.b1 = b1;
  a.t1 = (bf16*)t1;
  a.Ka = Ka;
  a.Kb = Kb;
  a.N1 = N1;
  a.N2 = N2;
  a.Ho = H, a.Wo = W, a.H2 = H2, a.W2 = W2, a.stride2 = stride2;
  a.fd_howo = fastdiv_make((uint32_t)(H * W));
  a.fd_wo = fastdiv_make((uint32_t)W);
  const long M = (long)B * H * W;
  const long sizes[7] = {M * Ka * 2, (long)B * H2 * W2 * Kb * 2, (long)N1 * (Ka + Kb) * 2, res ? M * N1 * 2 : 0,
                         M * N1 * 2, (long)N2 * N1 * 2, M * N2 * 2};
  for (long s : sizes)
    if (s >= 0x7fffffffL) return MLS_UNSUPPORTED;
  a.M = (int)M;
  a.t1in_bytes = (uint32_t)sizes[0];
  a.a2_bytes = (uint32_t)sizes[1];
  a.w3_bytes = (uint32_t)sizes[2];
  a.res_bytes = (uint32_t)sizes[3];
  a.y_bytes = (uint32_t)sizes[4];
  a.w1_bytes = (uint32_t)sizes[5];
  a.t1_bytes = (uint32_t)sizes[6];
  a.w2_bytes = 64 * 9 * 64 * 2;
  const hipStream_t st = (hipStream_t)stream;
  const int ks = (Ka + Kb) / 64;
  if (ks == 1 && N1 == 256 && N2 == 64) return launch_chain<1, 256, 64, 64, 128, true>(a, st);
  if (ks == 2 && N1 == 256 && N2 == 64) return launch_chain<2, 256, 64, 64, 128, true>(a, st);
  if (ks == 1 && N1 == 256 && N2 == 128) return launch_chain<1, 256, 128, 64, 128, true>(a, st);
  return MLS_UNSUPPORTED;
}

void mls_chain_set_l2_cw(int cw) { g_chain_cw_l2 = (cw == 32 || cw == 64) ? cw : 0; }

void mls_chain_set_l2_bm(int bm) { g_chain_bm_l2 = bm == 64 ? 64 : 128; }


void mls_chain_set_variant(int v) { g_chain_variant = (v == 1 || v == 2) ? v : 0; }

void mls_chain_set_grid(int g) { g_chain_grid = g > 0 ? g : 0; }

}

MLS_DEBUG_EXPORT(conv_chain)
```

### mlmicroservicetemplate_amd/ops/vision.py

```python
from __future__ import annotations

import ctypes
from typing import Optional, Tuple

import torch

from ._lib import check, lib, stream_ptr
from ._core import ACT_NONE, ACT_RELU, _act, _need, _ptr, _workspace_args, conv_out_hw


def pack_conv_weight(w_oihw: torch.Tensor, dtype=torch.bfloat16) -> torch.Tensor:
    co, ci, kh, kw = w_oihw.shape
    w = w_oihw.permute(0, 2, 3, 1)
    if ci == 3 and kh > 1:
        w = torch.nn.functional.pad(w, (0, 1, 0, 8 - kw))
    return w.contiguous().to(dtype)


CFG_HALO = 100


CFG_HALO_N32 = 101


CFG_HALO_XL = 102


HALO_CFGS = (CFG_HALO, CFG_HALO_N32, CFG_HALO_XL)


CFG_PIPE = 110


PIPE_VARIANTS = 12


PIPE_CFGS = tuple(range(CFG_PIPE, CFG_PIPE + PIPE_VARIANTS))


def conv2d_nhwc(
    x: torch.Tensor,
    w: torch.Tensor,
    bias: Optional[torch.Tensor] = None,
    *,
    kernel: int,
    stride: int = 1,
    pad: int = 0,
    scale: Optional[torch.Tensor] = None,
    residual: Optional[torch.Tensor] = None,
    act=ACT_NONE,
    out: Optional[torch.Tensor] = None,
    workspace: Optional[torch.Tensor] = None,
    cfg: int = 0,
    splitk: int = 0,
) -> torch.Tensor:
    dev = x.device
    _need(x, "x", torch.bfloat16, dev)
    _need(w, "w", torch.bfloat16, dev)
    B, H, W, C = x.shape
    cout = w.shape[0]
    kh = kw = kernel
    if C == 4 and kernel > 1:
        if tuple(w.shape) != (cout, kh, 8, 4):
            raise ValueError(f"stem weight must be [Cout,{kh},8,4], got {tuple(w.shape)}")
    elif tuple(w.shape) != (cout, kh, kw, C):
        raise ValueError(f"weight shape {tuple(w.shape)} != [{cout},{kh},{kw},{C}]")
    if cout % 8:
        raise ValueError("Cout must be a multiple of 8")
    ho, wo = conv_out_hw(H, W, kernel, stride, pad)
    if cfg in PIPE_CFGS:
        if kernel != 3 or stride != 1 or pad != 1 or scale is not None or residual is not None:
            raise ValueError("CFG_PIPE: 3x3 / stride 1 / pad 1 convolutions without a scale / residual only")
        ks, ipb = max(1, int(splitk)) % 16 or 1, max(1, int(splitk)) // 16 + 1
        return conv3x3_pipe(x, w, bias, act=act, out=out, variant=cfg - CFG_PIPE, splitk=ks, ipb=ipb,
                            workspace=workspace)
    if cfg in HALO_CFGS:
        if kernel != 3 or stride != 1 or pad != 1 or scale is not None:
            raise ValueError("CFG_HALO: 3x3 / stride 1 / pad 1 convolutions without a scale only")
        return conv3x3_halo(x, w, bias, act=act, residual=residual, out=out, variant=cfg - CFG_HALO,
                            splitk=splitk, workspace=workspace)
    for name, t in (("bias", bias), ("scale", scale)):
        if t is not None:
            _need(t, name, torch.float32, dev)
            if t.numel() != cout:
                raise ValueError(f"{name} must have {cout} elements")
    if residual is not None:
        _need(residual, "residual", torch.bfloat16, dev)
        if tuple(residual.shape) != (B, ho, wo, cout):
            raise ValueError(f"residual shape {tuple(residual.shape)} != {(B, ho, wo, cout)}")
    if out is None:
        out = torch.empty(B, ho, wo, cout, device=dev, dtype=torch.bfloat16)
    else:
        _need(out, "out", torch.bfloat16, dev)
        if tuple(out.shape) != (B, ho, wo, cout):
            raise ValueError("out has wrong shape")
    wsp, wsb = _workspace_args(workspace)
    rc = lib().mls_conv2d(
        x.data_ptr(), w.data_ptr(), _ptr(scale), _ptr(bias), _ptr(residual), out.data_ptr(), wsp, wsb,
        B, H, W, C, cout, kh, kw, stride, pad, _act(act), cfg, splitk, stream_ptr(dev),
    )
    check(rc, "mls_conv2d")
    return out


def conv1x1_dual(y: torch.Tensor, x: torch.Tensor, w_cat: torch.Tensor, bias: Optional[torch.Tensor] = None, *,
                 stride2: int = 1, act=ACT_NONE, out: Optional[torch.Tensor] = None,
                 workspace: Optional[torch.Tensor] = None, cfg: int = 0, splitk: int = 0) -> torch.Tensor:
    dev = y.device
    _need(y, "y", torch.bfloat16, dev)
    _need(x, "x", torch.bfloat16, dev)
    _need(w_cat, "w_cat", torch.bfloat16, dev)
    B, Ho, Wo, C1 = y.shape
    B2, H2, W2, C2 = x.shape
    cout = w_cat.shape[0]
    if B2 != B or tuple(w_cat.shape) != (cout, C1 + C2) or conv_out_hw(H2, W2, 1, stride2, 0) != (Ho, Wo):
        raise ValueError("conv1x1_dual: inconsistent shapes")
    if C1 % 64 or C2 % 8 or cout % 8:
        raise ValueError("conv1x1_dual needs Cin_y % 64 == 0, Cin_x % 8 == 0, Cout % 8 == 0")
    if bias is not None:
        _need(bias, "bias", torch.float32, dev)
    if out is None:
        out = torch.empty(B, Ho, Wo, cout, device=dev, dtype=torch.bfloat16)
    wsp, wsb = _workspace_args(workspace)
    rc = lib().mls_conv2d_dual(y.data_ptr(), x.data_ptr(), w_cat.data_ptr(), _ptr(bias), out.data_ptr(), wsp, wsb,
                               B, Ho, Wo, C1, H2, W2, C2, stride2, cout, _act(act), cfg, splitk, stream_ptr(dev))
    check(rc, "mls_conv2d_dual")
    return out


CHAIN_SHAPES = ((64, 256, 64), (128, 256, 64), (64, 256, 128), (128, 512, 128), (128, 512, 256), (256, 1024, 256))


def set_chain_l2_cw(cw: int) -> None:
    lib().mls_chain_set_l2_cw(int(cw))


def conv1x1_chain(a1: torch.Tensor, w3: torch.Tensor, b3: Optional[torch.Tensor], w1: torch.Tensor,
                  b1: Optional[torch.Tensor], *, residual: Optional[torch.Tensor] = None,
                  a2: Optional[torch.Tensor] = None, stride2: int = 1,
                  y_out: Optional[torch.Tensor] = None, t1_out: Optional[torch.Tensor] = None):
    dev = a1.device
    _need(a1, "a1", torch.bfloat16, dev)
    _need(w3, "w3", torch.bfloat16, dev)
    _need(w1, "w1", torch.bfloat16, dev)
    B, Ho, Wo, Ka = a1.shape
    N1, N2 = w3.shape[0], w1.shape[0]
    if a2 is not None:
        _need(a2, "a2", torch.bfloat16, dev)
        if residual is not None:
            raise ValueError("conv1x1_chain: the dual form has no residual")
        B2, H2, W2, Kb = a2.shape
        if B2 != B or conv_out_hw(H2, W2, 1, stride2, 0) != (Ho, Wo):
            raise ValueError("conv1x1_chain: a2 does not match a1's grid at stride2")
    else:
        H2 = W2 = Kb = 0
    if w3.reshape(N1, -1).shape[1] != Ka + Kb or w1.reshape(N2, -1).shape[1] != N1:
        raise ValueError("conv1x1_chain: weight shapes do not chain")
    if (Ka + Kb, N1, N2) not in CHAIN_SHAPES:
        raise ValueError(f"conv1x1_chain: unsupported shape (K {Ka + Kb}, N1 {N1}, N2 {N2})")
    for name, t, n in (("b3", b3, N1), ("b1", b1, N2)):
        if t is not None:
            _need(t, name, torch.float32, dev)
            if t.numel() != n:
                raise ValueError(f"{name} must have {n} elements")
    if residual is not None:
        _need(residual, "residual", torch.bfloat16, dev)
        if tuple(residual.shape) != (B, Ho, Wo, N1):
            raise ValueError("residual shape mismatch")
    y = torch.empty(B, Ho, Wo, N1, device=dev, dtype=torch.bfloat16) if y_out is None else y_out
    t1 = torch.empty(B, Ho, Wo, N2, device=dev, dtype=torch.bfloat16) if t1_out is None else t1_out
    rc = lib().mls_conv_chain(a1.data_ptr(), _ptr(a2), w3.data_ptr(), _ptr(b3), _ptr(residual), y.data_ptr(),
                              w1.data_ptr(), _ptr(b1), t1.data_ptr(), B, Ho, Wo, Ka, H2, W2, Kb, stride2, N1, N2,
                              stream_ptr(dev))
    check(rc, "mls_conv_chain")
    return y, t1


CHAIN_CONV2_SHAPES = ((0, 256, 64), (64, 256, 64), (0, 256, 128))
CHAIN_CONV2_MAX_W = 63


def conv3x3_chain(t1_in: torch.Tensor, w2: torch.Tensor, b2: Optional[torch.Tensor], w3: torch.Tensor,
                  b3: Optional[torch.Tensor], w1: torch.Tensor, b1: Optional[torch.Tensor], *,
                  residual: Optional[torch.Tensor] = None, a2: Optional[torch.Tensor] = None, stride2: int = 1,
                  y_out: Optional[torch.Tensor] = None, t1_out: Optional[torch.Tensor] = None):
    dev = t1_in.device
    for name, t in (("t1_in", t1_in), ("w2", w2), ("w3", w3), ("w1", w1)):
        _need(t, name, torch.bfloat16, dev)
    B, H, W, C = t1_in.shape
    N1, N2 = w3.shape[0], w1.shape[0]
    if C != 64 or tuple(w2.shape) != (64, 3, 3, 64):
        raise ValueError("conv3x3_chain: t1_in must be [B,H,W,64] and w2 [64,3,3,64]")
    Ka = 64
    if a2 is not None:
        _need(a2, "a2", torch.bfloat16, dev)
        if residual is not None:
            raise ValueError("conv3x3_chain: the dual form has no residual")
        B2, H2, W2, Kb = a2.shape
        if B2 != B or conv_out_hw(H2, W2, 1, stride2, 0) != (H, W):
            raise ValueError("conv3x3_chain: a2 does not match t1_in's grid at stride2")
    else:
        H2 = W2 = Kb = 0
    if w3.reshape(N1, -1).shape[1] != Ka + Kb or w1.reshape(N2, -1).shape[1] != N1:
        raise ValueError("conv3x3_chain: weight shapes do not chain")
    if (Kb, N1, N2) not in CHAIN_CONV2_SHAPES or W > CHAIN_CONV2_MAX_W:
        raise ValueError(f"conv3x3_chain: unsupported shape (Kb {Kb}, N1 {N1}, N2 {N2}, W {W})")
    for name, t, n in (("b2", b2, 64), ("b3", b3, N1), ("b1", b1, N2)):
        if t is not None:
            _need(t, name, torch.float32, dev)
            if t.numel() != n:
                raise ValueError(f"{name} must have {n} elements")
    if residual is not None:
        _need(residual, "residual", torch.bfloat16, dev)
        if tuple(residual.shape) != (B, H, W, N1):
            raise ValueError("residual shape mismatch")
    y = torch.empty(B, H, W, N1, device=dev, dtype=torch.bfloat16) if y_out is None else y_out
    t1 = torch.empty(B, H, W, N2, device=dev, dtype=torch.bfloat16) if t1_out is None else t1_out
    rc = lib().mls_conv_chain_conv2(t1_in.data_ptr(), w2.data_ptr(), _ptr(b2), _ptr(a2), w3.data_ptr(), _ptr(b3),
                                    _ptr(residual), y.data_ptr(), w1.data_ptr(), _ptr(b1), t1.data_ptr(), B, H, W,
                                    Ka, H2, W2, Kb, stride2, N1, N2, stream_ptr(dev))
    check(rc, "mls_conv_chain_conv2")
    return y, t1


_MEAN_STD_CACHE = {}


def normalize_u8(images: torch.Tensor, mean, std, pad: int = 0, out: Optional[torch.Tensor] = None) -> torch.Tensor:
    dev = images.device
    _need(images, "images", torch.uint8, dev)
    B, H, W, C = images.shape
    if C != 3:
        raise ValueError("expected 3-channel images")
    shape = (B, H + 2 * pad, W + 2 * pad, 4)
    if out is None:
        out = torch.empty(shape, device=dev, dtype=torch.bfloat16)
    else:
        _need(out, "out", torch.bfloat16, dev)
        if tuple(out.shape) != shape:
            raise ValueError(f"out must be {shape}")
    m = (ctypes.c_float * 3)(*[float(v) for v in mean])
    s = (ctypes.c_float * 3)(*[float(v) for v in std])
    rc = lib().mls_normalize_u8(images.data_ptr(), out.data_ptr(), B, H, W, pad, m, s, stream_ptr(dev))
    check(rc, "mls_normalize_u8")
    return out


def stem_pool_u8(images: torch.Tensor, w: torch.Tensor, bias: torch.Tensor, mean, std,
                 out: Optional[torch.Tensor] = None, conv1_w: Optional[torch.Tensor] = None,
                 conv1_b: Optional[torch.Tensor] = None):
    dev = images.device
    _need(images, "images", torch.uint8, dev)
    _need(w, "w", torch.bfloat16, dev)
    _need(bias, "bias", torch.float32, dev)
    B, H, W, C = images.shape
    if C != 3 or H != 224 or W != 224 or tuple(w.shape) != (64, 7, 8, 4) or bias.numel() != 64:
        raise ValueError("stem_pool_u8: 224x224x3 images, [64,7,8,4] weights, 64 biases")
    shape = (B, 56, 56, 64)
    if out is None:
        out = torch.empty(shape, device=dev, dtype=torch.bfloat16)
    else:
        _need(out, "out", torch.bfloat16, dev)
        if tuple(out.shape) != shape:
            raise ValueError(f"out must be {shape}")
    m = (ctypes.c_float * 3)(*[float(v) for v in mean])
    s = (ctypes.c_float * 3)(*[float(v) for v in std])
    if conv1_w is None:
        check(lib().mls_stem_pool(images.data_ptr(), w.data_ptr(), bias.data_ptr(), out.data_ptr(), B, H, W, m, s,
                                  stream_ptr(dev)), "mls_stem_pool")
        return out
    _need(conv1_w, "conv1_w", torch.bfloat16, dev)
    if conv1_w.numel() != 64 * 64 or conv1_w.shape[0] != 64:
        raise ValueError("stem_pool_u8: conv1_w must be [64, 64] (Cout x Cin)")
    if conv1_b is not None:
        _need(conv1_b, "conv1_b", torch.float32, dev)
        if conv1_b.numel() != 64:
            raise ValueError("conv1_b must have 64 elements")
    t1 = torch.empty(shape, device=dev, dtype=torch.bfloat16)
    check(lib().mls_stem_pool_conv1(images.data_ptr(), w.data_ptr(), bias.data_ptr(), out.data_ptr(), B, H, W, m, s,
                                    conv1_w.data_ptr(), _ptr(conv1_b), t1.data_ptr(), stream_ptr(dev)),
          "mls_stem_pool_conv1")
    return out, t1


def conv3x3_halo(x: torch.Tensor, w: torch.Tensor, bias: Optional[torch.Tensor] = None, *, act=ACT_NONE,
                 residual: Optional[torch.Tensor] = None, out: Optional[torch.Tensor] = None,
                 variant: int = 0, splitk: int = 1, workspace: Optional[torch.Tensor] = None) -> torch.Tensor:
    dev = x.device
    _need(x, "x", torch.bfloat16, dev)
    _need(w, "w", torch.bfloat16, dev)
    B, H, W, C = x.shape
    N = w.shape[0]
    if tuple(w.shape) != (N, 3, 3, C) or C % 32 or N % (32 if variant == 1 else 64) or variant not in (0, 1, 2):
        raise ValueError("conv3x3_halo: w must be [N,3,3,Cin], Cin % 32 == 0, N % 64 (variant 1: 32) == 0")
    if bias is not None:
        _need(bias, "bias", torch.float32, dev)
        if bias.numel() != N:
            raise ValueError("bias must have N elements")
    shape = (B, H, W, N)
    if residual is not None:
        _need(residual, "residual", torch.bfloat16, dev)
        if tuple(residual.shape) != shape:
            raise ValueError(f"residual must be {shape}")
    if out is None:
        out = torch.empty(shape, device=dev, dtype=torch.bfloat16)
    else:
        _need(out, "out", torch.bfloat16, dev)
        if tuple(out.shape) != shape:
            raise ValueError(f"out must be {shape}")
    wsp, wsb = _workspace_args(workspace)
    check(lib().mls_conv3x3_halo(x.data_ptr(), w.data_ptr(), _ptr(bias), _ptr(residual), out.data_ptr(), wsp, wsb,
                                 B, H, W, C, N, _act(act), variant, max(1, int(splitk)), stream_ptr(dev)),
          "mls_conv3x3_halo")
    return out


def conv2d_pool(x: torch.Tensor, w: torch.Tensor, bias: Optional[torch.Tensor], pool: torch.Tensor, *, kernel: int,
                stride: int = 1, pad: int = 0, residual: Optional[torch.Tensor] = None, act=ACT_NONE,
                out: Optional[torch.Tensor] = None, pool_only: bool = True, cfg: int = 0) -> Optional[torch.Tensor]:
    dev = x.device
    _need(x, "x", torch.bfloat16, dev)
    _need(w, "w", torch.bfloat16, dev)
    _need(pool, "pool", torch.float32, dev)
    B, H, W, C = x.shape
    cout = w.shape[0]
    if tuple(w.shape) != (cout, kernel, kernel, C) or C == 4:
        raise ValueError(f"weight shape {tuple(w.shape)} != [{cout},{kernel},{kernel},{C}]")
    ho, wo = conv_out_hw(H, W, kernel, stride, pad)
    if pool.shape[0] < B or pool.shape[-1] != cout:
        raise ValueError(f"pool must be [>= {B}, {cout}]")
    if bias is not None:
        _need(bias, "bias", torch.float32, dev)
    if residual is not None:
        _need(residual, "residual", torch.bfloat16, dev)
        if tuple(residual.shape) != (B, ho, wo, cout):
            raise ValueError("residual shape mismatch")
    if not pool_only and out is None:
        out = torch.empty(B, ho, wo, cout, device=dev, dtype=torch.bfloat16)
    check(lib().mls_conv2d_pool(x.data_ptr(), w.data_ptr(), None, _ptr(bias), _ptr(residual), _ptr(out),
                                pool.data_ptr(), int(pool_only), B, H, W, C, cout, kernel, kernel, stride, pad,
                                _act(act), int(cfg), stream_ptr(dev)), "mls_conv2d_pool")
    return out


def fc_head(pooled: torch.Tensor, w: torch.Tensor, bias: Optional[torch.Tensor], k: int, *,
            logits: Optional[torch.Tensor] = None, softmax: bool = True, err: Optional[torch.Tensor] = None,
            vals: Optional[torch.Tensor] = None, idx: Optional[torch.Tensor] = None):
    dev = pooled.device
    _need(pooled, "pooled", torch.float32, dev)
    _need(w, "w", torch.bfloat16, dev)
    B, K = pooled.shape
    N = w.shape[0]
    if w.shape[1] != K:
        raise ValueError("w must be [N, K]")
    if bias is not None:
        _need(bias, "bias", torch.float32, dev)
    if logits is None:
        logits = torch.empty(B, N, device=dev, dtype=torch.float32)
    _need(logits, "logits", torch.float32, dev)
    if logits.numel() < B * N:
        raise ValueError("logits buffer too small")
    if err is not None:
        _need(err, "err", torch.int32, dev)
    if k > 0:
        if vals is None:
            vals = torch.empty(B, k, device=dev, dtype=torch.float32)
        if idx is None:
            idx = torch.empty(B, k, device=dev, dtype=torch.int32)
    ws = torch.empty((K // 256) * B * N if K % 256 == 0 else 0, device=dev, dtype=torch.float32)
    check(lib().mls_fc_head(pooled.data_ptr(), w.data_ptr(), _ptr(bias), logits.data_ptr(), _ptr(vals), _ptr(idx),
                            _ptr(err), B, N, K, int(k), int(softmax), ws.data_ptr() if ws.numel() else None,
                            ws.numel() * 4, stream_ptr(dev)), "mls_fc_head")
    return vals, idx, logits


def conv3x3_pipe(x: torch.Tensor, w: torch.Tensor, bias: Optional[torch.Tensor] = None, *, act=ACT_NONE,
                 out: Optional[torch.Tensor] = None, variant: int = 0, splitk: int = 1, ipb: int = 1,
                 workspace: Optional[torch.Tensor] = None) -> torch.Tensor:
    dev = x.device
    _need(x, "x", torch.bfloat16, dev)
    _need(w, "w", torch.bfloat16, dev)
    B, H, W, C = x.shape
    N = w.shape[0]
    if tuple(w.shape) != (N, 3, 3, C) or C % 32 or N % 32 or N > 512 or not 0 <= variant < PIPE_VARIANTS:
        raise ValueError("conv3x3_pipe: w must be [N,3,3,Cin], Cin % 32 == 0, N % 32 == 0, N <= 512")
    if act not in (ACT_NONE, ACT_RELU, "none", "relu"):
        raise ValueError("conv3x3_pipe: act must be none or relu")
    if bias is not None:
        _need(bias, "bias", torch.float32, dev)
        if bias.numel() != N:
            raise ValueError("bias must have N elements")
    shape = (B, H, W, N)
    if out is None:
        out = torch.empty(shape, device=dev, dtype=torch.bfloat16)
    else:
        _need(out, "out", torch.bfloat16, dev)
        if tuple(out.shape) != shape:
            raise ValueError(f"out must be {shape}")
    wsp, wsb = _workspace_args(workspace)
    check(lib().mls_conv3x3_pipe(x.data_ptr(), w.data_ptr(), _ptr(bias), out.data_ptr(), wsp, wsb, B, H, W, C, N,
                                 _act(act), int(variant), max(1, int(splitk)), max(1, int(ipb)), stream_ptr(dev)),
          "mls_conv3x3_pipe")
    return out


def conv3x3_pipe_geometry(B: int, H: int, W: int, variant: int = 0) -> Optional[Tuple[int, int]]:
    th, nb = ctypes.c_int(0), ctypes.c_int(0)
    rc = lib().mls_conv3x3_pipe_geometry(B, H, W, variant, ctypes.byref(th), ctypes.byref(nb))
    return (th.value, nb.value) if rc == 0 else None


def conv3x3_halo_geometry(B: int, H: int, W: int, variant: int = 0) -> Optional[Tuple[int, int]]:
    th, nb = ctypes.c_int(0), ctypes.c_int(0)
    rc = lib().mls_conv3x3_halo_geometry_v(B, H, W, variant, ctypes.byref(th), ctypes.byref(nb))
    return (th.value, nb.value) if rc == 0 else None


def maxpool2d_nhwc(x: torch.Tensor, k: int = 3, s: int = 2, p: int = 1, out: Optional[torch.Tensor] = None):
    dev = x.device
    _need(x, "x", torch.bfloat16, dev)
    B, H, W, C = x.shape
    ho, wo = conv_out_hw(H, W, k, s, p)
    if out is None:
        out = torch.empty(B, ho, wo, C, device=dev, dtype=torch.bfloat16)
    rc = lib().mls_maxpool2d(x.data_ptr(), out.data_ptr(), B, H, W, C, k, s, p, stream_ptr(dev))
    check(rc, "mls_maxpool2d")
    return out


def avgpool_global_nhwc(x: torch.Tensor, out: Optional[torch.Tensor] = None) -> torch.Tensor:
    dev = x.device
    _need(x, "x", torch.bfloat16, dev)
    B, H, W, C = x.shape
    if out is None:
        out = torch.empty(B, C, device=dev, dtype=torch.bfloat16)
    rc = lib().mls_avgpool_global(x.data_ptr(), out.data_ptr(), B, H * W, C, stream_ptr(dev))
    check(rc, "mls_avgpool_global")
    return out


def bn_act(x: torch.Tensor, scale: torch.Tensor, bias: torch.Tensor, relu: bool = False, out=None) -> torch.Tensor:
    dev = x.device
    _need(x, "x", torch.bfloat16, dev)
    _need(scale, "scale", torch.float32, dev)
    _need(bias, "bias", torch.float32, dev)
    C = x.shape[-1]
    out = torch.empty_like(x) if out is None else out
    rc = lib().mls_bn_act(x.data_ptr(), out.data_ptr(), scale.data_ptr(), bias.data_ptr(), x.numel() // C, C,
                          int(relu), stream_ptr(dev))
    check(rc, "mls_bn_act")
    return out
```

Before: 58670 requests/s.

## Store only stride-2 subsampled block output when next downsample consumes it

When a chained bottleneck output feeds only the next stage's stride-2 1x1 downsample projection, the chain kernels now write just the even-row/even-column pixels of y. The downsample or dual conv then reads that compact tensor with stride 1. This cuts the y store traffic and the later strided read for the last block of layer1 and layer2. It adds new template instances, a per-thread precomputed output offset array, and new C entry points. It also relies on y having no other consumer, since the residual path of the next block is not used for first blocks.

```diff
diff --git a/mlmicroservicetemplate_amd/models/resnet.py b/mlmicroservicetemplate_amd/models/resnet.py
--- a/mlmicroservicetemplate_amd/models/resnet.py
+++ b/mlmicroservicetemplate_amd/models/resnet.py
@@ -278,6 +278,7 @@
         self.chain_conv2 = mode != "0"
         self.chain_conv2_shapes = ops.CHAIN_CONV2_SHAPES if mode == "2" else CHAIN_CONV2_DEFAULT
         self.chain_conv2_skip: set = {b for b in os.environ.get("MLS_CHAIN_CONV2_SKIP", "").split(",") if b}
+        self.chain_ysub = os.environ.get("MLS_CHAIN_YSUB", "1") != "0"
         self.chain_l3 = os.environ.get("MLS_CHAIN_L3", "0") == "1"
         if os.environ.get("MLS_CHAIN_L2_CW"):
             ops.set_chain_l2_cw(int(os.environ["MLS_CHAIN_L2_CW"]))
@@ -347,11 +348,11 @@
                     need = max(need, sk * M * N * 4)
         return max(need, batch * NUM_CLASSES * 4, 1 << 20)
 
-    def _conv(self, x, name, act, residual=None, pad=None):
+    def _conv(self, x, name, act, residual=None, pad=None, stride=None):
         s = self.specs[name]
         cfg, sk = self.tuning.get(name, (0, 0))
-        return self.ops.conv2d_nhwc(x, self.w[name], self.b[name], kernel=s.k, stride=s.stride,
-                                    pad=s.pad if pad is None else pad,
+        return self.ops.conv2d_nhwc(x, self.w[name], self.b[name], kernel=s.k,
+                                    stride=s.stride if stride is None else stride, pad=s.pad if pad is None else pad,
                                     residual=residual, act=act, workspace=self.workspace, cfg=cfg, splitk=sk)
 
 
@@ -365,6 +366,14 @@
         if shape == (256, 1024, 256) and not self.chain_l3:
             return False
         return c1.k == 1 and c1.stride == 1 and shape in self.ops.CHAIN_SHAPES
+
+    def _y_stride(self, p: str, nxt: str, dual: bool) -> int:
+        if not self.chain_ysub or not nxt.endswith(".0"):
+            return 1
+        c3, down = self.specs[p + ".conv3"], self.specs[nxt + ".down"]
+        k = c3.cin + (self.specs[p + ".down"].cin if dual else 0)
+        shape = (k, c3.cout, self.specs[nxt + ".conv1"].cout)
+        return 2 if down.k == 1 and down.stride == 2 and shape in self.ops.CHAIN_YSUB_SHAPES else 1
 
     def _conv2_fused(self, p: str, nxt: str, dual: bool, t1: torch.Tensor) -> bool:
         if not self.chain_conv2 or p in self.chain_conv2_skip:
@@ -422,22 +431,25 @@
                 x = ops.maxpool2d_nhwc(x, 3, 2, 1)
             t1 = self._conv(x, "layer1.0.conv1", ops.ACT_RELU)
         blocks = [(si, bi) for si, (nblocks, _m, _c, _s) in enumerate(STAGES) for bi in range(nblocks)]
+        xs = 1
         for idx, (si, bi) in enumerate(blocks):
             p = f"layer{si + 1}.{bi}"
             nxt = f"layer{blocks[idx + 1][0] + 1}.{blocks[idx + 1][1]}" if idx + 1 < len(blocks) else None
             dual = bi == 0 and self.fuse_down
             chained = nxt is not None and self._chained(p, nxt, dual)
+            ds = self.specs[p + ".down"].stride // xs if bi == 0 else 1
+            xs = self._y_stride(p, nxt, dual) if chained else 1
             if chained and self._conv2_fused(p, nxt, dual, t1):
                 w1n, b1n = self.w[nxt + ".conv1"], self.b[nxt + ".conv1"]
                 w1n = w1n.reshape(w1n.shape[0], -1)
                 w2, b2 = self.w[p + ".conv2"], self.b[p + ".conv2"]
                 if dual:
                     x, t1 = ops.conv3x3_chain(t1, w2, b2, self.dual_w[p], self.dual_b[p], w1n, b1n, a2=x,
-                                              stride2=self.specs[p + ".down"].stride)
+                                              stride2=ds, y_stride=xs)
                 else:
                     w3 = self.w[p + ".conv3"]
                     x, t1 = ops.conv3x3_chain(t1, w2, b2, w3.reshape(w3.shape[0], -1), self.b[p + ".conv3"], w1n,
-                                              b1n, residual=x)
+                                              b1n, residual=x, y_stride=xs)
                 continue
             t2 = self._conv(t1, p + ".conv2", ops.ACT_RELU)
             if chained:
@@ -445,18 +457,18 @@
                 w1n = w1n.reshape(w1n.shape[0], -1)
                 if dual:
                     x, t1 = ops.conv1x1_chain(t2, self.dual_w[p], self.dual_b[p], w1n, b1n, a2=x,
-                                              stride2=self.specs[p + ".down"].stride)
+                                              stride2=ds, y_stride=xs)
                 else:
                     w3 = self.w[p + ".conv3"]
                     x, t1 = ops.conv1x1_chain(t2, w3.reshape(w3.shape[0], -1), self.b[p + ".conv3"], w1n, b1n,
-                                              residual=x)
+                                              residual=x, y_stride=xs)
                 continue
             if dual:
                 cfg, sk = self.tuning.get(p + ".dual", (0, 0))
-                x = ops.conv1x1_dual(t2, x, self.dual_w[p], self.dual_b[p], stride2=self.specs[p + ".down"].stride,
-                                     act=ops.ACT_RELU, workspace=self.workspace, cfg=cfg, splitk=sk)
+                x = ops.conv1x1_dual(t2, x, self.dual_w[p], self.dual_b[p], stride2=ds, act=ops.ACT_RELU,
+                                     workspace=self.workspace, cfg=cfg, splitk=sk)
             else:
-                identity = self._conv(x, p + ".down", ops.ACT_NONE) if bi == 0 else x
+                identity = self._conv(x, p + ".down", ops.ACT_NONE, stride=ds) if bi == 0 else x
                 if nxt is None and pool:
                     pooled = self._pool.get()[: B * self.fc_w.shape[1]].view(B, -1)
                     cfg, _sk = self.tuning.get(p + ".conv3", (0, 0))
diff --git a/mlmicroservicetemplate_amd/ops/__init__.py b/mlmicroservicetemplate_amd/ops/__init__.py
--- a/mlmicroservicetemplate_amd/ops/__init__.py
+++ b/mlmicroservicetemplate_amd/ops/__init__.py
@@ -67,6 +67,7 @@
     CHAIN_CONV2_MAX_W,
     CHAIN_CONV2_SHAPES,
     CHAIN_SHAPES,
+    CHAIN_YSUB_SHAPES,
     HALO_CFGS,
     PIPE_CFGS,
     PIPE_VARIANTS,
diff --git a/mlmicroservicetemplate_amd/ops/_lib.py b/mlmicroservicetemplate_amd/ops/_lib.py
--- a/mlmicroservicetemplate_amd/ops/_lib.py
+++ b/mlmicroservicetemplate_amd/ops/_lib.py
@@ -25,6 +25,8 @@
     "mls_conv2d_dual": [P, P, P, P, P, P, SZ, I, I, I, I, I, I, I, I, I, I, I, I, P],
     "mls_conv_chain": [P, P, P, P, P, P, P, P, P, I, I, I, I, I, I, I, I, I, I, P],
     "mls_conv_chain_conv2": [P, P, P, P, P, P, P, P, P, P, P, I, I, I, I, I, I, I, I, I, I, P],
+    "mls_conv_chain_ys": [P, P, P, P, P, P, P, P, P, I, I, I, I, I, I, I, I, I, I, P, I],
+    "mls_conv_chain_conv2_ys": [P, P, P, P, P, P, P, P, P, P, P, I, I, I, I, I, I, I, I, I, I, P, I],
     "mls_gemm": [P, P, P, P, P, P, P, SZ, I, I, I, I, I, I, P],
     "mls_gemm_heuristic": [I, I, I, _c.POINTER(I), _c.POINTER(I)],
     "mls_gemm_tile": [P, P, P, P, P, I, I, I, I, I, I, I, I, I, P, _c.c_longlong, P, I, P],
diff --git a/mlmicroservicetemplate_amd/ops/csrc/conv_chain.hip b/mlmicroservicetemplate_amd/ops/csrc/conv_chain.hip
--- a/mlmicroservicetemplate_amd/ops/csrc/conv_chain.hip
+++ b/mlmicroservicetemplate_amd/ops/csrc/conv_chain.hip
@@ -45,13 +45,23 @@
   uint32_t t1in_bytes, w2_bytes;
 };
 
+template <int CPR, int N1>
+MLS_DEV int ysub_base(const ChainArgs& a, int m0, int q) {
+  const int m = m0 + q / CPR, c = q % CPR;
+  if (m >= a.M) return OOB;
+  const int b = fastdiv(m, a.fd_howo), rem = m - b * (a.Ho * a.Wo);
+  const int oh = fastdiv(rem, a.fd_wo), ow = rem - oh * a.Wo;
+  if ((oh | ow) & 1) return OOB;
+  return (((b * ((a.Ho + 1) >> 1) + (oh >> 1)) * ((a.Wo + 1) >> 1) + (ow >> 1)) * N1 + c * 8) * 2;
+}
+
 template <int CPR>
 MLS_DEV int row_swz(int r) {
   if constexpr (CPR == 8) return r & 7;
   else return (r & 1) | ((r >> 1) & 2);
 }
 
-template <int BM, int KS, int N1, int N2, int CW, int OCC, bool SW, bool C2 = false>
+template <int BM, int KS, int N1, int N2, int CW, int OCC, bool SW, bool C2 = false, int YS = 1>
 __global__ __launch_bounds__(512, OCC) void conv_chain_kernel(const ChainArgs a) {
   constexpr int NW = 8, NT = 512, WM = 4, WN = 2;
   constexpr int WTM = BM / WM, TM = WTM / 16;
@@ -81,6 +91,7 @@
   static_assert(W1_PW * NW * RPP == N2 && R_PW * NW * RPP == BM, "W1 / residual DMA split");
   static_assert(Y_ST * NT == BM * CPR && T_ST * NT == BM * N2 / 8, "epilogue split");
   static_assert(LDS_BYTES <= 160 * 1024, "LDS");
+  static_assert(YS == 1 || YS == 2, "y stride");
   __shared__ __attribute__((aligned(16))) char smem[LDS_BYTES];
 
   const int tid = threadIdx.x, lane = tid & 63;
@@ -269,6 +280,11 @@
     asm volatile("s_waitcnt lgkmcnt(0)" ::: "memory");
     __builtin_amdgcn_s_barrier();
   }
+  int ybase[Y_ST];
+  if constexpr (YS == 2) {
+#pragma unroll
+    for (int it = 0; it < Y_ST; ++it) ybase[it] = ysub_base<CPR, N1>(a, m0, tid + it * NT);
+  }
   issue(0, 0);
 
   f32x4 acc2[TM][TN2];
@@ -380,8 +396,10 @@
       const int row = q / CPR, c = q % CPR;
       const uint4 v = *reinterpret_cast<const uint4*>(sR + row * (CW * 2) + ((c ^ row_swz<CPR>(row)) << 4));
       const int m = m0 + row;
-      __builtin_amdgcn_raw_buffer_store_b128(__builtin_bit_cast(u32x4v, v), yr,
-                                             m < a.M ? (m * N1 + j * CW + c * 8) * 2 : OOB, 0, 0);
+      int off;
+      if constexpr (YS == 2) off = ybase[it] + j * CW * 2;
+      else off = m < a.M ? (m * N1 + j * CW + c * 8) * 2 : OOB;
+      __builtin_amdgcn_raw_buffer_store_b128(__builtin_bit_cast(u32x4v, v), yr, off, 0, 0);
     }
 
     const uint4* Ys = reinterpret_cast<const uint4*>(sR);
@@ -499,7 +517,7 @@
   asm volatile("ds_write_b16 %0, %1" ::"v"(off), "v"(v) : "memory");
 }
 
-template <int BM, int KS, int N1, int N2, int CW, int S, int OCC, bool SW, bool PERS>
+template <int BM, int KS, int N1, int N2, int CW, int S, int OCC, bool SW, bool PERS, int YS = 1>
 __global__ __launch_bounds__(512, OCC) void conv_chain_ring_kernel(const ChainArgs a, const int ntiles) {
   constexpr int NW = 8, NT = 512, WM = 4, WN = 2;
   constexpr int WTM = BM / WM, TM = WTM / 16;
@@ -525,6 +543,7 @@
   constexpr int T_ST = BM * N2 / 8 / NT;
   static_assert(TM >= 1 && TN >= 1 && TN2 >= 1 && (CW == 64 || CW == 32), "tile");
   static_assert(S >= 2 && S - 1 <= NJ && (!PERS || NJ % S == 0), "ring depth");
+  static_assert(YS == 1 || (YS == 2 && !PERS), "y stride");
   static_assert(Y_ST * NT == BM * CPR && T_ST * NT == BM * N2 / 8, "epilogue split");
   static_assert(LDS_BYTES <= 160 * 1024, "LDS");
   __shared__ __attribute__((aligned(16))) char smem[LDS_BYTES];
@@ -646,6 +665,12 @@
 #pragma unroll
     for (int jn = 0; jn < TN2; ++jn) acc2[i][jn] = f32x4{0.f, 0.f, 0.f, 0.f};
 
+  int ybase[Y_ST];
+  if constexpr (YS == 2) {
+#pragma unroll
+    for (int it = 0; it < Y_ST; ++it) ybase[it] = ysub_base<CPR, N1>(a, m0, tid + it * NT);
+  }
+
   int abuf = 0;
   bool first = true;
   for (;;) {
@@ -799,8 +824,10 @@
         const int row = q / CPR, c = q % CPR;
         const uint4 v = lds_ld16(lds_off(sR + row * (CW * 2) + ((c ^ row_swz<CPR>(row)) << 4)));
         const int m = m0 + row;
-        __builtin_amdgcn_raw_buffer_store_b128(__builtin_bit_cast(u32x4v, v), yr,
-                                               m < a.M ? (m * N1 + j * CW + c * 8) * 2 : OOB, 0, 0);
+        int off;
+        if constexpr (YS == 2) off = ybase[it] + j * CW * 2;
+        else off = m < a.M ? (m * N1 + j * CW + c * 8) * 2 : OOB;
+        __builtin_amdgcn_raw_buffer_store_b128(__builtin_bit_cast(u32x4v, v), yr, off, 0, 0);
       }
 
       const uint4* Ys = reinterpret_cast<const uint4*>(sR);
@@ -891,7 +918,7 @@
   if constexpr (PERS) asm volatile("s_waitcnt vmcnt(0)" ::: "memory");
 }
 
-template <int KS, int N1, int N2, int CW, int BM = 128, bool C2 = false>
+template <int KS, int N1, int N2, int CW, int BM = 128, bool C2 = false, int YS = 1>
 int launch_chain(const ChainArgs& a, hipStream_t st) {
   constexpr int LDS = BM * KS * 128 + 2 * (CW * KS * 128 + N2 * CW * 2 + BM * CW * 2);
   constexpr int OCC = LDS <= 80 * 1024 ? 4 : 2;
@@ -900,14 +927,14 @@
 #else
   constexpr bool SW = KS == 1;
 #endif
-  hipLaunchKernelGGL((conv_chain_kernel<BM, KS, N1, N2, CW, OCC, SW, C2>), dim3((unsigned)((a.M + BM - 1) / BM)),
+  hipLaunchKernelGGL((conv_chain_kernel<BM, KS, N1, N2, CW, OCC, SW, C2, YS>), dim3((unsigned)((a.M + BM - 1) / BM)),
                      dim3(512), 0, st, a);
   return (int)hipGetLastError();
 }
 
 int g_chain_grid = 0;
 
-template <int BM, int KS, int N1, int N2, int CW, int S, bool PERS>
+template <int BM, int KS, int N1, int N2, int CW, int S, bool PERS, int YS = 1>
 int launch_ring(const ChainArgs& a, hipStream_t st) {
 #ifdef MLS_CHAIN_SWAP
   constexpr bool SW = MLS_CHAIN_SWAP;
@@ -923,7 +950,7 @@
     const int cus = mls_num_cus();
     grid = g_chain_grid > 0 ? g_chain_grid : (ntiles < cus ? ntiles : cus);
   }
-  hipLaunchKernelGGL((conv_chain_ring_kernel<BM, KS, N1, N2, CW, S, OCC, SW, PERS>), dim3((unsigned)grid), dim3(512), 0,
+  hipLaunchKernelGGL((conv_chain_ring_kernel<BM, KS, N1, N2, CW, S, OCC, SW, PERS, YS>), dim3((unsigned)grid), dim3(512), 0,
                      st, a, ntiles);
   return (int)hipGetLastError();
 }
@@ -940,11 +967,12 @@
 
 extern "C" {
 
-int mls_conv_chain(const void* a1, const void* a2, const void* w3, const float* b3, const void* res, void* y,
-                   const void* w1, const float* b1, void* t1, int B, int Ho, int Wo, int Ka, int H2, int W2, int Kb,
-                   int stride2, int N1, int N2, void* stream) {
+int mls_conv_chain_ys(const void* a1, const void* a2, const void* w3, const float* b3, const void* res, void* y,
+                      const void* w1, const float* b1, void* t1, int B, int Ho, int Wo, int Ka, int H2, int W2, int Kb,
+                      int stride2, int N1, int N2, void* stream, int y_stride) {
   if (B <= 0 || Ho <= 0 || Wo <= 0 || Ka <= 0 || Ka % 64 || Kb < 0 || Kb % 64 || N1 <= 0 || N1 % 64 || N2 <= 0)
     return MLS_BAD_ARG;
+  if (y_stride != 1 && y_stride != 2) return MLS_BAD_ARG;
   if (Kb > 0 && (stride2 < 1 || (Ho - 1) * stride2 >= H2 || (Wo - 1) * stride2 >= W2 || res)) return MLS_BAD_ARG;
   ChainArgs a{};
   a.a1 = (const bf16*)a1;
@@ -965,8 +993,9 @@
   a.fd_howo = fastdiv_make((uint32_t)(Ho * Wo));
   a.fd_wo = fastdiv_make((uint32_t)Wo);
   const long M = a.M;
+  const long My = y_stride == 2 ? (long)B * ((Ho + 1) / 2) * ((Wo + 1) / 2) : M;
   const long sizes[7] = {M * Ka * 2, (long)B * H2 * W2 * Kb * 2, (long)N1 * (Ka + Kb) * 2, res ? M * N1 * 2 : 0,
-                         M * N1 * 2, (long)N2 * N1 * 2, M * N2 * 2};
+                         My * N1 * 2, (long)N2 * N1 * 2, M * N2 * 2};
   for (long s : sizes)
     if (s >= 0x7fffffffL) return MLS_UNSUPPORTED;
   a.a1_bytes = (uint32_t)sizes[0];
@@ -978,12 +1007,21 @@
   a.t1_bytes = (uint32_t)sizes[6];
   const hipStream_t st = (hipStream_t)stream;
   const int ks = (Ka + Kb) / 64;
+  const bool l2_override = g_chain_variant == 0 && (g_chain_bm_l2 == 64 || g_chain_cw_l2 != 0);
+  if (y_stride == 2) {
+    if (ks == 1 && N1 == 256 && N2 == 128) return launch_chain<1, 256, 128, 64, 128, false, 2>(a, st);
+    if (ks == 2 && N1 == 512 && N2 == 256) {
+      if (!l2_override && use_ring(RING_L2_OUT)) return launch_ring<128, 2, 512, 256, 32, 3, false, 2>(a, st);
+      return g_chain_bm_l2 == 64 ? launch_chain<2, 512, 256, 64, 64, false, 2>(a, st)
+                                 : launch_chain<2, 512, 256, 32, 128, false, 2>(a, st);
+    }
+    return MLS_UNSUPPORTED;
+  }
   if (ks == 1 && N1 == 256 && N2 == 64) return launch_chain<1, 256, 64, 64>(a, st);
   if (ks == 2 && N1 == 256 && N2 == 64)
     return use_ring(RING_L1_DUAL) ? launch_ring<64, 2, 256, 64, 64, 2, true>(a, st)
                                   : launch_chain<2, 256, 64, 64>(a, st);
   if (ks == 1 && N1 == 256 && N2 == 128) return launch_chain<1, 256, 128, 64>(a, st);
-  const bool l2_override = g_chain_variant == 0 && (g_chain_bm_l2 == 64 || g_chain_cw_l2 != 0);
   if (ks == 2 && N1 == 512 && N2 == 128) {
     if (!l2_override && use_ring(RING_L2)) return launch_ring<128, 2, 512, 128, 64, 2, false>(a, st);
     if (g_chain_bm_l2 == 64) return launch_chain<2, 512, 128, 64, 64>(a, st);
@@ -997,10 +1035,18 @@
   return MLS_UNSUPPORTED;
 }
 
-int mls_conv_chain_conv2(const void* t1_in, const void* w2, const float* b2, const void* a2, const void* w3,
-                         const float* b3, const void* res, void* y, const void* w1, const float* b1, void* t1, int B,
-                         int H, int W, int Ka, int H2, int W2, int Kb, int stride2, int N1, int N2, void* stream) {
+int mls_conv_chain(const void* a1, const void* a2, const void* w3, const float* b3, const void* res, void* y,
+                   const void* w1, const float* b1, void* t1, int B, int Ho, int Wo, int Ka, int H2, int W2, int Kb,
+                   int stride2, int N1, int N2, void* stream) {
+  return mls_conv_chain_ys(a1, a2, w3, b3, res, y, w1, b1, t1, B, Ho, Wo, Ka, H2, W2, Kb, stride2, N1, N2, stream, 1);
+}
+
+int mls_conv_chain_conv2_ys(const void* t1_in, const void* w2, const float* b2, const void* a2, const void* w3,
+                            const float* b3, const void* res, void* y, const void* w1, const float* b1, void* t1,
+                            int B, int H, int W, int Ka, int H2, int W2, int Kb, int stride2, int N1, int N2,
+                            void* stream, int y_stride) {
   if (B <= 0 || H <= 0 || W <= 0 || Ka <= 0 || Kb < 0 || Kb % 64 || N1 <= 0 || N1 % 64 || N2 <= 0) return MLS_BAD_ARG;
+  if (y_stride != 1 && y_stride != 2) return MLS_BAD_ARG;
   if (Kb > 0 && (stride2 < 1 || (H - 1) * stride2 >= H2 || (W - 1) * stride2 >= W2 || res)) return MLS_BAD_ARG;
   if (Ka != 64 || 2 * (W + 1) + 128 > 256) return MLS_UNSUPPORTED;
   ChainArgs a{};
@@ -1023,8 +1069,9 @@
   a.fd_howo = fastdiv_make((uint32_t)(H * W));
   a.fd_wo = fastdiv_make((uint32_t)W);
   const long M = (long)B * H * W;
+  const long My = y_stride == 2 ? (long)B * ((H + 1) / 2) * ((W + 1) / 2) : M;
   const long sizes[7] = {M * Ka * 2, (long)B * H2 * W2 * Kb * 2, (long)N1 * (Ka + Kb) * 2, res ? M * N1 * 2 : 0,
-                         M * N1 * 2, (long)N2 * N1 * 2, M * N2 * 2};
+                         My * N1 * 2, (long)N2 * N1 * 2, M * N2 * 2};
   for (long s : sizes)
     if (s >= 0x7fffffffL) return MLS_UNSUPPORTED;
   a.M = (int)M;
@@ -1038,12 +1085,21 @@
   a.w2_bytes = 64 * 9 * 64 * 2;
   const hipStream_t st = (hipStream_t)stream;
   const int ks = (Ka + Kb) / 64;
+  if (y_stride == 2)
+    return ks == 1 && N1 == 256 && N2 == 128 ? launch_chain<1, 256, 128, 64, 128, true, 2>(a, st) : MLS_UNSUPPORTED;
   if (ks == 1 && N1 == 256 && N2 == 64) return launch_chain<1, 256, 64, 64, 128, true>(a, st);
   if (ks == 2 && N1 == 256 && N2 == 64) return launch_chain<2, 256, 64, 64, 128, true>(a, st);
   if (ks == 1 && N1 == 256 && N2 == 128) return launch_chain<1, 256, 128, 64, 128, true>(a, st);
   return MLS_UNSUPPORTED;
 }
 
+int mls_conv_chain_conv2(const void* t1_in, const void* w2, const float* b2, const void* a2, const void* w3,
+                         const float* b3, const void* res, void* y, const void* w1, const float* b1, void* t1, int B,
+                         int H, int W, int Ka, int H2, int W2, int Kb, int stride2, int N1, int N2, void* stream) {
+  return mls_conv_chain_conv2_ys(t1_in, w2, b2, a2, w3, b3, res, y, w1, b1, t1, B, H, W, Ka, H2, W2, Kb, stride2, N1,
+                                 N2, stream, 1);
+}
+
 void mls_chain_set_l2_cw(int cw) { g_chain_cw_l2 = (cw == 32 || cw == 64) ? cw : 0; }
 
 void mls_chain_set_l2_bm(int bm) { g_chain_bm_l2 = bm == 64 ? 64 : 128; }
diff --git a/mlmicroservicetemplate_amd/ops/vision.py b/mlmicroservicetemplate_amd/ops/vision.py
--- a/mlmicroservicetemplate_amd/ops/vision.py
+++ b/mlmicroservicetemplate_amd/ops/vision.py
@@ -129,16 +129,27 @@
 
 
 CHAIN_SHAPES = ((64, 256, 64), (128, 256, 64), (64, 256, 128), (128, 512, 128), (128, 512, 256), (256, 1024, 256))
+CHAIN_YSUB_SHAPES = ((64, 256, 128), (128, 512, 256))
 
 
 def set_chain_l2_cw(cw: int) -> None:
     lib().mls_chain_set_l2_cw(int(cw))
+
+
+def _chain_y(y_out: Optional[torch.Tensor], B: int, Ho: int, Wo: int, N1: int, y_stride: int, dev) -> torch.Tensor:
+    shape = (B, -(-Ho // y_stride), -(-Wo // y_stride), N1)
+    if y_out is None:
+        return torch.empty(shape, device=dev, dtype=torch.bfloat16)
+    _need(y_out, "y_out", torch.bfloat16, dev)
+    if tuple(y_out.shape) != shape:
+        raise ValueError(f"y_out must be {shape}, got {tuple(y_out.shape)}")
+    return y_out
 
 
 def conv1x1_chain(a1: torch.Tensor, w3: torch.Tensor, b3: Optional[torch.Tensor], w1: torch.Tensor,
                   b1: Optional[torch.Tensor], *, residual: Optional[torch.Tensor] = None,
                   a2: Optional[torch.Tensor] = None, stride2: int = 1,
-                  y_out: Optional[torch.Tensor] = None, t1_out: Optional[torch.Tensor] = None):
+                  y_out: Optional[torch.Tensor] = None, t1_out: Optional[torch.Tensor] = None, y_stride: int = 1):
     dev = a1.device
     _need(a1, "a1", torch.bfloat16, dev)
     _need(w3, "w3", torch.bfloat16, dev)
@@ -158,6 +169,10 @@
         raise ValueError("conv1x1_chain: weight shapes do not chain")
     if (Ka + Kb, N1, N2) not in CHAIN_SHAPES:
         raise ValueError(f"conv1x1_chain: unsupported shape (K {Ka + Kb}, N1 {N1}, N2 {N2})")
+    if y_stride not in (1, 2):
+        raise ValueError("conv1x1_chain: y_stride must be 1 or 2")
+    if y_stride == 2 and (Ka + Kb, N1, N2) not in CHAIN_YSUB_SHAPES:
+        raise ValueError(f"conv1x1_chain: no y_stride = 2 form for (K {Ka + Kb}, N1 {N1}, N2 {N2})")
     for name, t, n in (("b3", b3, N1), ("b1", b1, N2)):
         if t is not None:
             _need(t, name, torch.float32, dev)
@@ -167,12 +182,12 @@
         _need(residual, "residual", torch.bfloat16, dev)
         if tuple(residual.shape) != (B, Ho, Wo, N1):
             raise ValueError("residual shape mismatch")
-    y = torch.empty(B, Ho, Wo, N1, device=dev, dtype=torch.bfloat16) if y_out is None else y_out
+    y = _chain_y(y_out, B, Ho, Wo, N1, y_stride, dev)
     t1 = torch.empty(B, Ho, Wo, N2, device=dev, dtype=torch.bfloat16) if t1_out is None else t1_out
-    rc = lib().mls_conv_chain(a1.data_ptr(), _ptr(a2), w3.data_ptr(), _ptr(b3), _ptr(residual), y.data_ptr(),
-                              w1.data_ptr(), _ptr(b1), t1.data_ptr(), B, Ho, Wo, Ka, H2, W2, Kb, stride2, N1, N2,
-                              stream_ptr(dev))
-    check(rc, "mls_conv_chain")
+    rc = lib().mls_conv_chain_ys(a1.data_ptr(), _ptr(a2), w3.data_ptr(), _ptr(b3), _ptr(residual), y.data_ptr(),
+                                 w1.data_ptr(), _ptr(b1), t1.data_ptr(), B, Ho, Wo, Ka, H2, W2, Kb, stride2, N1, N2,
+                                 stream_ptr(dev), y_stride)
+    check(rc, "mls_conv_chain_ys")
     return y, t1
 
 
@@ -183,7 +198,7 @@
 def conv3x3_chain(t1_in: torch.Tensor, w2: torch.Tensor, b2: Optional[torch.Tensor], w3: torch.Tensor,
                   b3: Optional[torch.Tensor], w1: torch.Tensor, b1: Optional[torch.Tensor], *,
                   residual: Optional[torch.Tensor] = None, a2: Optional[torch.Tensor] = None, stride2: int = 1,
-                  y_out: Optional[torch.Tensor] = None, t1_out: Optional[torch.Tensor] = None):
+                  y_out: Optional[torch.Tensor] = None, t1_out: Optional[torch.Tensor] = None, y_stride: int = 1):
     dev = t1_in.device
     for name, t in (("t1_in", t1_in), ("w2", w2), ("w3", w3), ("w1", w1)):
         _need(t, name, torch.bfloat16, dev)
@@ -205,6 +220,10 @@
         raise ValueError("conv3x3_chain: weight shapes do not chain")
     if (Kb, N1, N2) not in CHAIN_CONV2_SHAPES or W > CHAIN_CONV2_MAX_W:
         raise ValueError(f"conv3x3_chain: unsupported shape (Kb {Kb}, N1 {N1}, N2 {N2}, W {W})")
+    if y_stride not in (1, 2):
+        raise ValueError("conv3x3_chain: y_stride must be 1 or 2")
+    if y_stride == 2 and (Ka + Kb, N1, N2) not in CHAIN_YSUB_SHAPES:
+        raise ValueError(f"conv3x3_chain: no y_stride = 2 form for (Kb {Kb}, N1 {N1}, N2 {N2})")
     for name, t, n in (("b2", b2, 64), ("b3", b3, N1), ("b1", b1, N2)):
         if t is not None:
             _need(t, name, torch.float32, dev)
@@ -214,12 +233,12 @@
         _need(residual, "residual", torch.bfloat16, dev)
         if tuple(residual.shape) != (B, H, W, N1):
             raise ValueError("residual shape mismatch")
-    y = torch.empty(B, H, W, N1, device=dev, dtype=torch.bfloat16) if y_out is None else y_out
+    y = _chain_y(y_out, B, H, W, N1, y_stride, dev)
     t1 = torch.empty(B, H, W, N2, device=dev, dtype=torch.bfloat16) if t1_out is None else t1_out
-    rc = lib().mls_conv_chain_conv2(t1_in.data_ptr(), w2.data_ptr(), _ptr(b2), _ptr(a2), w3.data_ptr(), _ptr(b3),
-                                    _ptr(residual), y.data_ptr(), w1.data_ptr(), _ptr(b1), t1.data_ptr(), B, H, W,
-                                    Ka, H2, W2, Kb, stride2, N1, N2, stream_ptr(dev))
-    check(rc, "mls_conv_chain_conv2")
+    rc = lib().mls_conv_chain_conv2_ys(t1_in.data_ptr(), w2.data_ptr(), _ptr(b2), _ptr(a2), w3.data_ptr(), _ptr(b3),
+                                       _ptr(residual), y.data_ptr(), w1.data_ptr(), _ptr(b1), t1.data_ptr(), B, H, W,
+                                       Ka, H2, W2, Kb, stride2, N1, N2, stream_ptr(dev), y_stride)
+    check(rc, "mls_conv_chain_conv2_ys")
     return y, t1
 
 
```

Result: faster. 59670 requests/s (median of 6 runs) (+1.7%).
